# ecrireme/ESR-NeRF

Hardware: AMD Instinct MI355X
Metric: training rays/sec at 4096 rays x 128 samples (fine stage) (higher is better)
Workload: dtype f32; 1 GPU; C2: giftbox_w fine stage on the slab scene, 4096 rays x 128 samples per GPU, grid 256x256x64, s_val=20, forward + trainer loss + backward + the TV lines on every third step (no optimizer step); rays_per_gpu=4096, samples_per_ray=128, surviving_samples=524288, parallelism=dp1

## Files before the change

### esr_nerf_amd/_lib.py

```python
from __future__ import annotations

import ctypes as C
import os

import torch

_HERE = os.path.dirname(os.path.abspath(__file__))
LIB_PATH = os.path.join(_HERE, "libesr_hip.so")
LIB_PATH = os.environ.get("ESR_LIB_PATH", LIB_PATH)
ABI_VERSION = 29
_lib = None


class EsrScene(C.Structure):
    _fields_ = [
        ("xyz_min", C.c_float * 3), ("xyz_max", C.c_float * 3),
        ("mask_min", C.c_float * 3), ("mask_max", C.c_float * 3),
        ("gx", C.c_int32), ("gy", C.c_int32), ("gz", C.c_int32),
        ("mx", C.c_int32), ("my", C.c_int32), ("mz", C.c_int32),
        ("near_", C.c_float), ("stepdist", C.c_float), ("voxel_size", C.c_float),
        ("act_shift", C.c_float), ("mask_thres", C.c_float), ("fast_thres", C.c_float),
        ("s_val", C.c_float), ("max_steps", C.c_int32), ("grad_feat", C.c_float * 4),
    ]


class EsrPlan(C.Structure):
    _fields_ = [(n, C.c_int32) for n in
                ("n_on", "n_off", "tiles_on", "tiles_all", "m0", "m1", "m2", "overflow")]


class EsrFeatArgs(C.Structure):
    _fields_ = [(n, C.c_void_p) for n in ("rays_o", "rays_d", "viewdirs", "rec_ray", "rec_step", "rec_sdf",
                                          "pts", "pt_viewdirs", "pt_sdf")] + \
               [("n_pts", C.c_int32), ("sdf", C.c_void_p), ("color_on", C.c_void_p * 3),
                ("color_off", C.c_void_p * 3), ("tiles_on", C.c_int32), ("tiles_all", C.c_int32)]


class EsrFeatBwdSrc(C.Structure):
    _fields_ = [("dX", C.c_void_p), ("grad_color_on", C.c_void_p), ("grad_color_off", C.c_void_p),
                ("t0", C.c_int32), ("t1", C.c_int32)]


class EsrLtsArgs(C.Structure):
    _fields_ = [("n_pts", C.c_int32), ("n_rays", C.c_int32), ("n_sg", C.c_int32), ("pdra_mode", C.c_int32)] + \
               [(n, C.c_void_p) for n in ("base", "rough", "metal", "normal", "view", "dirs", "off_m", "emo_m",
                                          "last2", "mus", "lambdas", "lobes", "emission", "umask")]


class EsrLtsGather(C.Structure):
    _fields_ = [(n, C.c_void_p) for n in ("jp", "ray64", "pts_all", "eg", "rec_sdf", "viewdirs", "brdf_a", "emit_a",
                                          "umask_rays")] + [("n_pts", C.c_int32)] + \
               [(n, C.c_void_p) for n in ("pts2", "vd2", "sdf2", "normal", "base", "rough", "metal", "emis", "umask", "pt1")]


class EsrActJob(C.Structure):
    _fields_ = [("z", C.c_void_p), ("g_tile", C.c_void_p), ("out", C.c_void_p), ("tiles", C.c_int32), ("rows", C.c_int32),
                ("n_ch", C.c_int32), ("act", C.c_int32), ("bwd", C.c_int32), ("src", C.c_void_p), ("src_c", C.c_int32),
                ("n_src", C.c_int32), ("inv", C.c_void_p), ("pt1", C.c_void_p), ("ex", C.c_void_p * 3),
                ("ex_c", C.c_int32 * 3), ("ex_col0", C.c_int32 * 3)]


class EsrGatherJob(C.Structure):
    _fields_ = [("src", C.c_void_p), ("tile_rows", C.c_int32), ("row_stride", C.c_int32), ("col0", C.c_int32),
                ("n_ch", C.c_int32), ("perm", C.c_void_p), ("n", C.c_int32), ("out", C.c_void_p)]


class EsrPairJob(C.Structure):
    _fields_ = [("a", C.c_void_p), ("b", C.c_void_p), ("rows", C.c_int64), ("cols", C.c_int32), ("row_mask", C.c_void_p),
                ("mask_value", C.c_int32), ("count_dev", C.c_void_p), ("kind", C.c_int32), ("w_value", C.c_float),
                ("w_a", C.c_float), ("w_b", C.c_float), ("ga", C.c_void_p), ("gb", C.c_void_p)]


class EsrLtsGrads(C.Structure):
    _fields_ = [(n, C.c_void_p) for n in ("d_off_m", "d_emo_m", "d_last2", "d_base", "d_rough", "d_metal",
                                          "d_emission", "d_mus", "d_lambdas", "d_lobes")]


class EsrCdIndex(C.Structure):
    _fields_ = [("origin", C.c_double * 3), ("h", C.c_double), ("dims", C.c_int32 * 3), ("coarse", C.c_int32),
                ("cap", C.c_int64), ("keys", C.c_void_p), ("cells", C.c_void_p), ("start", C.c_void_p), ("pts", C.c_void_p),
                ("ids", C.c_void_p), ("ccap", C.c_int64), ("ckeys", C.c_void_p)]


class EsrDvgo(C.Structure):
    _fields_ = [("density", C.c_void_p), ("off_color", C.c_void_p), ("emo_color", C.c_void_p), ("dims", C.c_int32 * 3),
                ("xyz_min", C.c_float * 3), ("xyz_max", C.c_float * 3)] + \
               [(n, C.c_float) for n in ("near_", "far_", "step_scale", "interval", "act_shift")] + [("n_samples", C.c_int32)]


class EsrDvgoRays(C.Structure):
    _fields_ = [(n, C.c_void_p) for n in ("rays_o", "rays_d", "nrm", "jitter", "em_modes")] + \
               [("em_all", C.c_int32), ("n_rays", C.c_int64)]


class EsrDvgoOut(C.Structure):
    _fields_ = [(n, C.c_void_p) for n in ("alpha", "alphainv_cum", "weights", "raw_rgb", "rgb", "depth", "disp", "white_bg",
                                          "off_rgb", "on_rgb", "emo_rgb")]


class EsrDvgoBwd(C.Structure):
    _fields_ = [(n, C.c_void_p) for n in ("alpha", "alphainv_cum", "raw_rgb", "g_alphainv_cum", "g_weights", "g_raw_rgb",
                                          "g_rgb", "grad_density", "grad_off", "grad_emo")]


class EsrMlpWeights(C.Structure):
    _fields_ = [("w", C.c_void_p * 4), ("b", C.c_void_p * 4)]


class EsrWgradJob(C.Structure):
    _fields_ = [("kind", C.c_int32), ("color_row0", C.c_int32), ("t0", C.c_int32), ("t1", C.c_int32),
                ("X", C.c_void_p), ("H", C.c_void_p), ("dZ", C.c_void_p), ("dz", C.c_void_p),
                ("gw", C.c_void_p), ("gb", C.c_void_p), ("X16", C.c_void_p), ("amax", C.c_void_p)]


EXPORTS = [
    "esr_abi_version", "esr_build_info",
    "esr_sample_count", "esr_sample_fill", "esr_alpha2weight_fwd", "esr_alpha2weight_bwd",
    "esr_tv_add_grad", "esr_segment_sum",
    "esr_sample_count_f64", "esr_sample_fill_f64", "esr_alpha2weight_fwd_f64", "esr_alpha2weight_bwd_f64",
    "esr_infer_t_minmax", "esr_infer_n_samples", "esr_infer_ray_start_dir", "esr_sample_ndc_pts", "esr_sample_bg_pts",
    "esr_maskcache_lookup", "esr_raw2alpha", "esr_raw2alpha_bwd", "esr_tv_add_grad_masked",
    "esr_fine_march_count", "esr_fine_plan_begin", "esr_fine_plan", "esr_fine_plan_totals", "esr_fine_plan_offsets", "esr_fine_march_fill",
    "esr_fine_march_bwd", "esr_fine_march_bwd_rec", "esr_fine_march_cache_floats", "esr_fine_march_count_cached",
    "esr_fine_march_fill_cached", "esr_fine_march_bwd_cached", "esr_fine_march_count_ga", "esr_fine_march_fill_ga", "esr_fine_march_bwd_ga",
    "esr_fine_feat_fwd", "esr_fine_feat_fwd_x16", "esr_fine_feat_x16_bytes", "esr_fine_feat_bwd",
    "esr_mlp_packed_floats", "esr_mlp_pack", "esr_mlp_pack_batch", "esr_mlp_packed_split_elems", "esr_mlp_split_gain_offset", "esr_mlp_split_range_flag", "esr_mlp_fwd_split", "esr_mlp_fwd_fine_split", "esr_mlp_dgrad_split", "esr_mlp_dgrad_fine_split", "esr_absmax", "esr_mlp_fwd", "esr_mlp_fwd_mixed", "esr_mlp_fwd_fine", "esr_mlp_dgrad_fine", "esr_mlp_fwd_fine_bf16", "esr_mlp_dgrad_fine_bf16", "esr_mlp_dgrad", "esr_mlp_wgrad", "esr_mlp_wgrad_batch", "esr_tone_wgrad_scratch_floats", "esr_tone_wgrad_recompute", "esr_tone_wgrad_recompute_bf16", "esr_tone_wgrad_recompute_split",
    "esr_mlp_wgrad_scratch_floats",
    "esr_fine_tone_in_fwd", "esr_fine_composite_fwd", "esr_fine_composite_bwd",
    "esr_fine_tone_in_bwd", "esr_fine_loss_fwd_bwd_dp",
    "esr_expgrad_fwd", "esr_expgrad_bwd", "esr_lts_dirs", "esr_lts_ref_order", "esr_lts_perturb", "esr_lts_gather_rows",
    "esr_lts_gather_points", "esr_lts_combine_fwd", "esr_lts_combine_bwd",
    "esr_act_fwd", "esr_act_bwd", "esr_act_batch", "esr_lts_gather_rows_batch", "esr_pair_loss_batch", "esr_lts_ref_order_inv", "esr_lts_dirs_rays", "esr_composite3_fwd", "esr_composite3_bwd", "esr_lts_tone_in_bwd",
    "esr_sample_points", "esr_pair_loss_fwd_bwd", "esr_emit_edit",
    "esr_gauss3d_fwd", "esr_gauss3d_bwd", "esr_central_grad_fwd", "esr_central_grad_bwd",
    "esr_coarse_march_count", "esr_coarse_march_fill", "esr_coarse_march_bwd", "esr_coarse_march_count_ga", "esr_coarse_march_fill_ga", "esr_coarse_march_bwd_ga",
    "esr_coarse_feat_fwd", "esr_coarse_feat_bwd", "esr_coarse_shade_fwd", "esr_coarse_shade_bwd",
    "esr_adam_step", "esr_eval_aux", "esr_eval_disp",
    "esr_mlp_packed_bf16_elems", "esr_mlp_pack_bf16", "esr_mlp_fwd_bf16", "esr_mlp_dgrad_bf16", "esr_mlp_wgrad_bf16",
    "esr_brick_floats", "esr_brick_flags", "esr_brick_pack", "esr_brick_unpack", "esr_brick_list", "esr_brick_list_scratch_ints",
    "esr_smooth_grad_tv_fwd", "esr_smooth_grad_tv_bwd", "esr_host_choice_noreplace", "esr_host_choice_start", "esr_host_choice_wait",
    "esr_mesh_field", "esr_mesh_blocks", "esr_mesh_count", "esr_mesh_emit",
    "esr_cd_sample_count", "esr_cd_sample_fill", "esr_cd_cell_keys", "esr_cd_hash_insert", "esr_cd_downsample_round",
    "esr_cd_nn",
    "esr_dvgo_fwd", "esr_dvgo_eval", "esr_dvgo_bwd", "esr_dvgo_count", "esr_dvgo_count_add",
]


def lib() -> C.CDLL:
    global _lib
    if _lib is None:
        if not os.path.exists(LIB_PATH):
            raise RuntimeError(
                f"{LIB_PATH} is missing: build it with `python -m esr_nerf_amd.build` "
                "(there is no CPU fallback for the HIP path)")
        L = C.CDLL(LIB_PATH)
        L.esr_abi_version.restype = C.c_int
        L.esr_build_info.restype = C.c_char_p
        if hasattr(L, "esr_mlp_packed_floats"):
            L.esr_mlp_packed_floats.restype = C.c_int64
            L.esr_mlp_wgrad_scratch_floats.restype = C.c_int64
            L.esr_tone_wgrad_scratch_floats.restype = C.c_int64
            L.esr_fine_march_cache_floats.restype = C.c_int64
        if hasattr(L, "esr_fine_feat_x16_bytes"):
            L.esr_fine_feat_x16_bytes.restype = C.c_int64
        if hasattr(L, "esr_brick_list_scratch_ints"):
            L.esr_brick_list_scratch_ints.restype = C.c_int64
        if hasattr(L, "esr_mlp_packed_bf16_elems"):
            L.esr_mlp_packed_bf16_elems.restype = C.c_int64
        if hasattr(L, "esr_mlp_packed_split_elems"):
            L.esr_mlp_packed_split_elems.restype = C.c_int64
        if hasattr(L, "esr_mlp_split_gain_offset"):
            L.esr_mlp_split_gain_offset.restype = C.c_int64
        if hasattr(L, "esr_mesh_blocks"):
            L.esr_mesh_blocks.restype = C.c_int64
        for name in ("esr_cd_sample_count", "esr_cd_sample_fill", "esr_cd_cell_keys", "esr_cd_hash_insert",
                     "esr_cd_downsample_round", "esr_cd_nn"):
            if hasattr(L, name):
                getattr(L, name).restype = C.c_int
        if L.esr_abi_version() != ABI_VERSION:
            raise RuntimeError("libesr_hip.so ABI version mismatch: rebuild")
        _lib = L
    return _lib


def check(code: int, what: str):
    if code != 0:
        raise RuntimeError(f"{what} failed with code {code}" +
                           (" (hipError)" if code > 0 else
                            " (a capacity limit of the kernels is exceeded, include/esr_hip.h: ESR_ECAP)" if code == -2 else
                            " (bad argument)"))


def ptr(t):
    if t is None:
        return C.c_void_p(0)
    if not t.is_cuda:
        raise RuntimeError("esr_hip ops need device tensors (got a CPU tensor)")
    if not t.is_contiguous():
        raise RuntimeError("esr_hip ops need contiguous tensors")
    return C.c_void_p(t.data_ptr())


_dev_index = {}


def stream_ptr(device=None):
    idx = _dev_index.get(device)
    if idx is None:
        idx = torch.cuda.current_device() if device is None else torch.device(device).index
        if idx is None:
            idx = torch.cuda.current_device()
        elif device is not None:
            _dev_index[device] = idx
    return C.c_void_p(torch._C._cuda_getCurrentRawStream(idx))


def ptr_array(tensors, n=None):
    n = n or len(tensors)
    arr = (C.c_void_p * n)()
    for i, t in enumerate(tensors):
        arr[i] = 0 if t is None else t.data_ptr()
    return arr
```

### esr_nerf_amd/build.py

```python
from __future__ import annotations

import concurrent.futures as cf
import hashlib
import os
import shlex
import subprocess
import sys

HERE = os.path.dirname(os.path.abspath(__file__))
CSRC = os.path.join(HERE, "csrc")
OBJ = os.path.join(HERE, "_obj")
LIB = os.path.join(HERE, "libesr_hip.so")
HEADER = os.path.join(os.path.dirname(HERE), "include", "esr_hip.h")
VARIANTS = os.path.join(os.path.dirname(HERE), "tools", "_variants")
HIPCC = os.environ.get("HIPCC", "/opt/rocm/bin/hipcc")
ARCH = "gfx950"
NO_PACKED_FP32 = ["-Xclang", "-target-feature", "-Xclang", "-packed-fp32-ops"]
FLAGS = ["-O3", "-std=c++17", "-fPIC", f"--offload-arch={ARCH}", "-fvisibility=hidden",
         "-Wall", "-Wno-unused-function", "-fno-fast-math", *NO_PACKED_FP32]


EXTRA = {"tone_wgrad.hip": ["-fno-slp-vectorize"], "mlp_split.hip": ["-mllvm", "-amdgpu-mfma-vgpr-form=1"]}


def hipcc_cmd(src, extra=()):
    return [HIPCC, *FLAGS, *EXTRA.get(src, []), *extra]


def sources():
    return sorted(f for f in os.listdir(CSRC) if f.endswith(".hip"))


def _make(src, out, args):
    h = hashlib.sha1(" ".join(hipcc_cmd(src, args)[1:]).encode())
    for p in sorted([os.path.join(CSRC, src), HEADER] + [os.path.join(CSRC, f) for f in os.listdir(CSRC) if f.endswith(".h")]):
        with open(p, "rb") as f:
            h.update(f.read())
    stamp, sfile = h.hexdigest(), out + ".stamp"
    if os.path.exists(out) and os.path.exists(sfile) and open(sfile).read() == stamp:
        return False
    r = subprocess.run([*hipcc_cmd(src, args), os.path.join(CSRC, src), "-o", out], capture_output=True, text=True)
    if r.returncode != 0:
        raise RuntimeError(f"hipcc failed for {src}:\n{r.stdout}\n{r.stderr}")
    noise = ("'-packed-fp32-ops' is not a recognized feature", "argument unused during compilation: '--hip-link'")
    err = "\n".join(l for l in r.stderr.splitlines() if not any(n in l for n in noise))
    if err.strip():
        sys.stderr.write(err + "\n")
    with open(sfile, "w") as f:
        f.write(stamp)
    return True


def _compile(src, extra=(), obj=None):
    obj = obj or os.path.join(OBJ, src[:-4] + ".o")
    return obj, _make(src, obj, [*extra, "-c"])


def _link(objs, lib):
    r = subprocess.run([HIPCC, "-shared", "-fPIC", f"--offload-arch={ARCH}", "-o", lib, *objs], capture_output=True, text=True)
    if r.returncode != 0:
        raise RuntimeError(f"link failed:\n{r.stdout}\n{r.stderr}")


def build_lib(force: bool = False, jobs: int = 4) -> str:
    os.makedirs(OBJ, exist_ok=True)
    if force:
        for f in os.listdir(OBJ):
            os.remove(os.path.join(OBJ, f))
    with cf.ThreadPoolExecutor(max_workers=jobs) as ex:
        res = list(ex.map(_compile, sources()))
    if any(changed for _, changed in res) or not os.path.exists(LIB):
        _link([o for o, _ in res], LIB)
    return LIB


def build_variant(name, src, extra=()) -> str:
    if src not in sources():
        raise ValueError(f"no source csrc/{src}")
    build_lib()
    os.makedirs(VARIANTS, exist_ok=True)
    obj, _ = _compile(src, extra, os.path.join(VARIANTS, name + ".o"))
    lib = os.path.join(VARIANTS, name + ".so")
    _link([obj if s == src else os.path.join(OBJ, s[:-4] + ".o") for s in sources()], lib)
    return lib


def device_asm(src) -> str:
    os.makedirs(OBJ, exist_ok=True)
    out = os.path.join(OBJ, src[:-4] + ".s")
    _make(src, out, ["-S", "--cuda-device-only"])
    return out


if __name__ == "__main__":
    args = sys.argv[1:]
    if args[:1] == ["--variant"] and len(args) >= 3:
        print(build_variant(args[1], args[2], args[3:]))
    elif args[:1] == ["--flags"] and len(args) == 2:
        print(shlex.join(hipcc_cmd(args[1])[1:]))
    elif args in ([], ["--force"]):
        print(build_lib(force=bool(args)))
    else:
        sys.exit(__doc__)
```

### esr_nerf_amd/fine_engine.py

```python
from __future__ import annotations

import ctypes as C
import functools
import math
import os
from dataclasses import dataclass
from typing import Dict, List, Optional

import torch

from . import _lib

KIND_RADIANCE, KIND_TONEMAP = 0, 1
HID = 192
X_ROWS, DX_ROWS, XT_ROWS = 104, 64, 48


def make_scene(xyz_min, xyz_max, mask_min, mask_max, world_size, mask_size, near, stepdist,
               voxel_size, act_shift, mask_thres, fast_thres, s_val, grad_feat) -> _lib.EsrScene:
    sc = _lib.EsrScene()
    for i in range(3):
        sc.xyz_min[i], sc.xyz_max[i] = float(xyz_min[i]), float(xyz_max[i])
        sc.mask_min[i], sc.mask_max[i] = float(mask_min[i]), float(mask_max[i])
    sc.gx, sc.gy, sc.gz = [int(v) for v in world_size]
    sc.mx, sc.my, sc.mz = [int(v) for v in mask_size]
    sc.near_, sc.stepdist, sc.voxel_size = float(near), float(stepdist), float(voxel_size)
    sc.act_shift, sc.mask_thres, sc.fast_thres = float(act_shift), float(mask_thres), float(fast_thres)
    sc.s_val = float(s_val)
    diag = math.sqrt(sum((float(xyz_max[i]) - float(xyz_min[i])) ** 2 for i in range(3)))
    sc.max_steps = int(diag / float(stepdist)) + 4
    if len(grad_feat) != 4:
        raise NotImplementedError("the HIP feature kernel is built for 4 stencil radii (cfg grad_feat)")
    for i in range(4):
        sc.grad_feat[i] = float(grad_feat[i])
    return sc


_RANGE_FLAGS = {}


@dataclass
class FineCtx:
    scene: _lib.EsrScene
    n_rays: int
    tiles_on: int
    tiles_all: int
    counts: Dict[str, int]
    rays_o: torch.Tensor
    rays_d: torch.Tensor
    viewdirs: torch.Tensor
    off3: torch.Tensor
    mask_density: torch.Tensor
    sdf: torch.Tensor
    feat_args: object = None
    march_cache: object = None
    x16: bool = False
    f32_only: bool = False


class _Workspace:

    def __init__(self, device):
        self.device = device
        self.cap_tiles = 0
        self.buf: Dict[str, torch.Tensor] = {}

    ROWS = dict(X=X_ROWS, gnorm=4, H0=HID, H1=HID, H2=HID, z_off=4, z_emo=4, lin=4, Xt=XT_ROWS, Ht=HID,
                zt=4, rgb=4, dzt=4, dZt=HID, dXt=DX_ROWS, dz=4, dZ0=HID, dZ1=HID, dZ2=HID, dX=DX_ROWS,
                dweight=1, rec_w=1, rec_sdf=1, dsdf=1)

    def ensure(self, tiles: int):
        if tiles <= self.cap_tiles:
            return
        cap = int(max(tiles, self.cap_tiles) * 1.25) + 64
        self.buf = {k: torch.empty(cap * r * 32, dtype=torch.float32, device=self.device)
                    for k, r in self.ROWS.items()}
        for k in ("M0", "M1", "M2", "Mt"):
            self.buf[k] = torch.empty(cap * 3 * 64, dtype=torch.int32, device=self.device)
        self.buf["rec_ray"] = torch.empty(cap * 32, dtype=torch.int32, device=self.device)
        self.buf["rec_step"] = torch.empty(cap * 32, dtype=torch.int32, device=self.device)
        self.buf["X16"] = torch.empty(cap * 26 * 256, dtype=torch.uint8, device=self.device)
        self.cap_tiles = cap

    def __getitem__(self, k):
        return self.buf[k]


class _F32Only:
    def __init__(self, eng):
        self.eng = eng

    def __enter__(self):
        self.keep, self.eng.split_fwd = self.eng.split_fwd, False

    def __exit__(self, *exc):
        self.eng.split_fwd = self.keep
        return False


def _follows_forward(backward):
    @functools.wraps(backward)
    def run(self, ctx, *args, **kw):
        if ctx.f32_only and self.split_fwd:
            with self.f32_only():
                return backward(self, ctx, *args, **kw)
        return backward(self, ctx, *args, **kw)
    return run


class _PackGroup:
    def __init__(self, eng):
        self.eng = eng

    def __enter__(self):
        self.eng._pack_pending = []

    def __exit__(self, et, ev, tb):
        eng = self.eng
        jobs, eng._pack_pending = eng._pack_pending, None
        if et is None and jobs:
            eng._pack_flush(jobs)
        return False


class FineEngine:
    def __init__(self, device, mlp_dtype: str = "f32"):
        if mlp_dtype not in ("f32", "bf16"):
            raise ValueError("mlp_dtype must be 'f32' or 'bf16'")
        self.device = torch.device(device)
        self.bf16 = mlp_dtype == "bf16"
        self.packed16: Dict[str, torch.Tensor] = {}
        self._p16: Dict[int, C.c_void_p] = {}
        self.L = _lib.lib()
        self.ws = _Workspace(self.device)
        self.plan_dev = torch.zeros(8, dtype=torch.int32, device=self.device)
        self.plan_host = torch.zeros(8, dtype=torch.int32).pin_memory()
        self.packed = {
            k: torch.empty(self.L.esr_mlp_packed_floats(kind), dtype=torch.float32, device=self.device)
            for k, kind in (("off", KIND_RADIANCE), ("emo", KIND_RADIANCE), ("tone", KIND_TONEMAP))}
        self.ray_bufs: Dict[int, Dict[str, torch.Tensor]] = {}
        self.wgrad_scratch = torch.empty(self.L.esr_mlp_wgrad_scratch_floats(), dtype=torch.float32,
                                         device=self.device)
        self._timing = False
        self._only = None
        self._events = []
        self.n_calls = 0
        self.overlap_wgrad = True
        self._side = None
        self._raw: Dict[str, tuple] = {}
        self._pack_cache: Dict[str, tuple] = {}
        self._pack_pending = None
        self._pack_batch_cache = None
        self.x16 = self.bf16
        self.split_fwd = (not self.bf16) and os.environ.get("ESR_SPLIT_FWD", "1") != "0"
        self.split_strict = os.environ.get("ESR_SPLIT_STRICT", "0") == "1"
        self.split_fallback_steps = 0
        self.packed_split: Dict[str, torch.Tensor] = {}
        self._psplit = {}
        self.range_flag = None
        self._range_host = None
        self._range_event = None
        if self.split_fwd:
            key = str(self.device)
            if key not in _RANGE_FLAGS:
                _RANGE_FLAGS[key] = torch.zeros(1, dtype=torch.int32, device=self.device)
            self.range_flag = _RANGE_FLAGS[key]
            self._range_host = torch.zeros(1, dtype=torch.int32).pin_memory()
            with torch.cuda.device(self.device):
                _lib.check(self.L.esr_mlp_split_range_flag(_lib.ptr(self.range_flag)), "esr_mlp_split_range_flag")
        self.tone_scratch = torch.empty(self.L.esr_tone_wgrad_scratch_floats(), dtype=torch.float32, device=self.device)
        self.neus_grad = False

    def _s(self):
        return _lib.stream_ptr(self.device)

    defer_overflow = False
    overflow_seen = False
    range_strict_seen = False
    _range_streak = 0

    split_kinds = split_kinds_bwd = frozenset({0, 1, 2, 3})
    last_draws = None

    def _split_phase(self, on):
        if bool(on) != self.split_fwd:
            raise AttributeError("every split-fp16 launch follows split_fwd: set split_fwd instead")

    split_bwd = split_wgrad = split_tone_wgrad = property(lambda self: self.split_fwd, _split_phase)

    def _overflow(self):
        if not self.defer_overflow:
            raise RuntimeError("a ray exceeded scene.max_steps; the LDS bound of the march kernel is wrong")
        self.overflow_seen = True

    _RANGE_MSG = ("an input, a hidden activation or a weight of an MLP left fp16's range (|x| >= 60000, |w| >= 1023, inf / NaN) in a "
                  "split-fp16 kernel (csrc/mlp_split.hip)")

    def range_probe(self):
        if self.range_flag is None or not self.split_fwd:
            self._range_event = None
            return
        self._range_host.copy_(self.range_flag, non_blocking=True)
        self._range_event = torch.cuda.Event()
        self._range_event.record()

    def range_hit(self) -> bool:
        ev, self._range_event = self._range_event, None
        if ev is None:
            return False
        ev.synchronize()
        if int(self._range_host[0]) == 0:
            self._range_streak = 0
            return False
        self.range_flag.zero_()
        if self.split_strict:
            if self.defer_overflow:
                self.overflow_seen = True
                self.range_strict_seen = True
                return False
            raise RuntimeError(self._RANGE_MSG + " (ESR_SPLIT_STRICT=1: no fallback)")
        import warnings
        if self.split_fallback_steps == 0:
            warnings.warn(self._RANGE_MSG + ": the step is re-run on the f32 MFMA kernels (slower; counted in "
                          "engine.split_fallback_steps)", RuntimeWarning, stacklevel=3)
        self.split_fallback_steps += 1
        self._range_streak += 1
        if self._range_streak >= self.RANGE_STREAK_MAX and self.split_fwd:
            self.split_fwd = False
            warnings.warn(f"{self.RANGE_STREAK_MAX} consecutive steps left fp16's range: this engine now runs every MLP launch on the "
                          "f32 MFMA kernels (as with ESR_SPLIT_FWD=0)", RuntimeWarning, stacklevel=3)
        return True

    RANGE_STREAK_MAX = 3

    def f32_only(self):
        return _F32Only(self)

    def healed(self, run, rerun=None):
        self._range_event = None
        out = run()
        if self.range_hit():
            with self.f32_only():
                out = (rerun or run)()
        return out

    def _run(self, name, fn, *args):
        self.n_calls += 1
        if self._timing and (self._only is None or name in self._only):
            e0 = torch.cuda.Event(enable_timing=True)
            e1 = torch.cuda.Event(enable_timing=True)
            e0.record()
            rc = fn(*args)
            e1.record()
            self._events.append((name, e0, e1))
        else:
            rc = fn(*args)
        _lib.check(rc, name)

    def enable_timing(self, on: bool, only=None):
        self._timing = bool(on)
        self._only = set(only) if only is not None else None
        self._events = []

    def timing_summary(self):
        torch.cuda.synchronize(self.device)
        out = {}
        for name, e0, e1 in self._events:
            n, ms = out.get(name, (0, 0.0))
            out[name] = (n + 1, ms + e0.elapsed_time(e1))
        return out

    def _march(self, name, which, sp, rays_o, rays_d, viewdirs, *rest):
        if self.neus_grad:
            fn = getattr(self.L, f"esr_fine_march_{which}_ga")
            self._run(name, fn, sp, _lib.ptr(rays_o), _lib.ptr(rays_d), _lib.ptr(viewdirs), *rest)
        else:
            self._run(name, getattr(self.L, f"esr_fine_march_{which}"), sp, _lib.ptr(rays_o), _lib.ptr(rays_d), *rest)

    def _ray_buf(self, n, scene=None):
        if n not in self.ray_bufs:
            self.ray_bufs[n] = dict(
                cnt3=torch.empty(n, dtype=torch.int32, device=self.device),
                off3=torch.empty(n, dtype=torch.int32, device=self.device),
                stats=torch.empty(n * 3, dtype=torch.int32, device=self.device))
        rb = self.ray_bufs[n]
        if scene is not None:
            need = int(self.L.esr_fine_march_cache_floats(C.byref(scene), n))
            if rb.get("cache") is None or rb["cache"].numel() < need:
                rb["cache"] = torch.empty(need, dtype=torch.float32, device=self.device)
        return rb

    def pack(self, which: str, kind: int, weights: List[torch.Tensor], biases: List[torch.Tensor]):
        self._raw[which] = (list(weights), list(biases))
        key = tuple((t.data_ptr(), t.dtype, t.numel(), t.is_contiguous()) for t in weights) + \
            tuple((t.data_ptr(), t.dtype, t.numel(), t.is_contiguous()) for t in biases)
        hit = self._pack_cache.get(which)
        if hit is None or hit[0] != key or hit[1] != kind or hit[6] != self.packed[which].data_ptr():
            w = _lib.EsrMlpWeights()
            for i, (a, b) in enumerate(zip(weights, biases)):
                if not (a.is_cuda and b.is_cuda and a.is_contiguous() and b.is_contiguous()
                        and a.dtype == torch.float32 and b.dtype == torch.float32):
                    raise RuntimeError("MLP parameters must be contiguous fp32 device tensors")
                w.w[i], w.b[i] = a.data_ptr(), b.data_ptr()
            p32 = _lib.ptr(self.packed[which])
            p16 = None
            if self.bf16:
                n16 = self.L.esr_mlp_packed_bf16_elems(kind)
                if which not in self.packed16 or self.packed16[which].numel() != n16:
                    self.packed16[which] = torch.empty(n16, dtype=torch.bfloat16, device=self.device)
                p16 = _lib.ptr(self.packed16[which])
                self._p16[self.packed[which].data_ptr()] = p16
            if self.split_fwd and kind in self.split_kinds:
                ns = self.L.esr_mlp_packed_split_elems(kind)
                if which not in self.packed_split or self.packed_split[which].numel() != ns:
                    self.packed_split[which] = torch.empty(ns, dtype=torch.float16, device=self.device)
                self._psplit[self.packed[which].data_ptr()] = _lib.ptr(self.packed_split[which])
            hit = self._pack_cache[which] = (key, kind, w, C.byref(w), p32, p16, self.packed[which].data_ptr())
        _, _, w, wref, p32, p16, _ = hit
        if self._pack_pending is not None:
            self._pack_pending.append((which, kind, w, p32, p16))
            return
        if self.split_fwd and kind in self.split_kinds:
            return self._pack_flush([(which, kind, w, p32, p16)])
        s = self._s()
        self._run(f"mlp_pack({which})", self.L.esr_mlp_pack, kind, wref, p32, s)
        if self.bf16:
            self._run(f"mlp_pack16({which})", self.L.esr_mlp_pack_bf16, kind, wref, p16, s)

    def packing(self):
        return _PackGroup(self)

    def _pack_flush(self, jobs):
        split = [(self.packed_split[which].data_ptr() if (self.split_fwd and kind in self.split_kinds) else 0)
                 for which, kind, _, _, _ in jobs]
        sig = tuple((which, kind, C.addressof(w), p32.value, p16.value if p16 is not None else 0, sp)
                    for (which, kind, w, p32, p16), sp in zip(jobs, split))
        hit = self._pack_batch_cache
        if hit is None or hit[0] != sig:
            n = len(jobs)
            kinds = (C.c_int32 * n)(*[k for _, k, _, _, _ in jobs])
            ws = (C.c_void_p * n)(*[C.addressof(w) for _, _, w, _, _ in jobs])
            p32s = (C.c_void_p * n)(*[p.value for _, _, _, p, _ in jobs])
            p16s = (C.c_void_p * n)(*[(p.value if p is not None else 0) for _, _, _, _, p in jobs]) if self.bf16 else None
            psp = (C.c_void_p * n)(*split) if any(split) else None
            hit = self._pack_batch_cache = (sig, n, kinds, ws, p32s, p16s, psp)
        _, n, kinds, ws, p32s, p16s, psp = hit
        self._run("mlp_pack(all)", self.L.esr_mlp_pack_batch, n, kinds, ws, p32s, p16s, psp, self._s())

    def mlp_fwd(self, kind, packed, *rest):
        if not self.bf16:
            planes = self._psplit.get(packed.value) if self.split_fwd else None
            if planes is not None:
                return self.L.esr_mlp_fwd_split(kind, packed, planes, *rest)
            return self.L.esr_mlp_fwd(kind, packed, *rest)
        return self.L.esr_mlp_fwd_bf16(kind, packed, self._p16[packed.value], *rest)

    def mlp_dgrad(self, kind, packed, *rest):
        if not self.bf16:
            planes = self._psplit.get(packed.value) if self.split_fwd else None
            if planes is not None:
                return self.L.esr_mlp_dgrad_split(kind, planes, *rest[:-1], None, rest[-1])
            return self.L.esr_mlp_dgrad(kind, packed, *rest)
        return self.L.esr_mlp_dgrad_bf16(kind, self._p16[packed.value], *rest)

    def mlp_wgrad(self, *args):
        return (self.L.esr_mlp_wgrad_bf16 if self.bf16 else self.L.esr_mlp_wgrad)(*args)

    def _H(self, names):
        return _lib.ptr_array([self.ws[n] for n in names])

    def feat_args(self, rays_o, rays_d, viewdirs, sdf, tiles_on, tiles_all, color_on, color_off, ws=None):
        ws = ws or self.ws
        fa = _lib.EsrFeatArgs()
        fa.rays_o, fa.rays_d, fa.viewdirs = rays_o.data_ptr(), rays_d.data_ptr(), viewdirs.data_ptr()
        fa.rec_ray, fa.rec_step, fa.rec_sdf = ws["rec_ray"].data_ptr(), ws["rec_step"].data_ptr(), ws["rec_sdf"].data_ptr()
        fa.sdf = sdf.data_ptr()
        for g in range(3):
            fa.color_on[g] = color_on[g].data_ptr() if color_on[g] is not None else None
            fa.color_off[g] = color_off[g].data_ptr() if color_off[g] is not None else None
        fa.tiles_on, fa.tiles_all = tiles_on, tiles_all
        return fa

    def forward(self, scene, rays_o, rays_d, viewdirs, em_modes, mask_density, sdf, off_color, emo_color, prelude=None,
                heal: bool = True):
        run = lambda: self._forward(scene, rays_o, rays_d, viewdirs, em_modes, mask_density, sdf, off_color, emo_color, prelude)
        return self.healed(run) if heal else run()

    def _forward(self, scene, rays_o, rays_d, viewdirs, em_modes, mask_density, sdf, off_color, emo_color, prelude=None):
        L, s, ws = self.L, self._s(), self.ws
        n = rays_o.shape[0]
        for t in (rays_o, rays_d, viewdirs):
            if t.dtype != torch.float32:
                raise RuntimeError("rays must be fp32")
        if em_modes.dtype != torch.int64:
            raise RuntimeError("em_modes must be int64")
        cached = not self.neus_grad
        rb = self._ray_buf(n, scene if cached else None)
        last = torch.empty(n, dtype=torch.float32, device=self.device)
        n3 = (3 * n + 3) // 4 * 4
        zb = torch.zeros(8 + 2 * n3 + 4, dtype=torch.float32, device=self.device)
        plan_dev = zb[:8].view(torch.int32)
        srgb, lin = zb[8: 8 + 3 * n].view(n, 3), zb[8 + n3: 8 + n3 + 3 * n].view(n, 3)
        self._loss_acc = zb[8 + 2 * n3: 8 + 2 * n3 + 2]
        self._amax = zb[8 + 2 * n3 + 3: 8 + 2 * n3 + 4]
        self._amax_t = zb[8 + 2 * n3 + 2: 8 + 2 * n3 + 3]
        sp = C.byref(scene)
        main = torch.cuda.current_stream(self.device)
        if cached:
            self._run("march_count", L.esr_fine_march_count_cached, sp, _lib.ptr(rays_o), _lib.ptr(rays_d), _lib.ptr(mask_density),
                      _lib.ptr(sdf), n, _lib.ptr(rb["cnt3"]), _lib.ptr(last), _lib.ptr(rb["stats"]), _lib.ptr(plan_dev),
                      _lib.ptr(rb["cache"]), s)
        else:
            self._march("march_count", "count", sp, rays_o, rays_d, viewdirs, _lib.ptr(mask_density),
                        _lib.ptr(sdf), n, _lib.ptr(rb["cnt3"]), _lib.ptr(last), _lib.ptr(rb["stats"]), _lib.ptr(plan_dev), s)
        self._run("plan_totals", L.esr_fine_plan_totals, _lib.ptr(rb["cnt3"]), _lib.ptr(em_modes), _lib.ptr(rb["stats"]), n,
                  _lib.ptr(plan_dev), s)
        self.plan_host.copy_(plan_dev, non_blocking=True)
        landed = torch.cuda.Event()
        landed.record()
        self._run("plan", L.esr_fine_plan_offsets, _lib.ptr(rb["cnt3"]), _lib.ptr(em_modes), n, _lib.ptr(rb["off3"]), _lib.ptr(plan_dev), s)
        e_pre = None
        if prelude is not None:
            side = self._side_stream(0)
            side.wait_event(landed)
            with torch.cuda.stream(side):
                prelude()
                e_pre = torch.cuda.Event()
                e_pre.record(side)
        pre_rec = ws.buf.get("rec_ray")
        if pre_rec is not None:
            pre_rec.fill_(-1)
        landed.synchronize()
        n_on, n_off, _, _, m0, m1, m2, overflow = [int(v) for v in self.plan_host.tolist()]
        tiles_on = (n_on + 31) // 32
        tiles_all = tiles_on + (n_off + 31) // 32
        if overflow & 1:
            self._overflow()
        ctx = FineCtx(scene=scene, n_rays=n, tiles_on=tiles_on, tiles_all=tiles_all,
                      counts=dict(m0=m0, m1=m1, m2=m2, m3=n_on + n_off, n_on=n_on, n_off=n_off),
                      rays_o=rays_o, rays_d=rays_d, viewdirs=viewdirs, off3=rb["off3"], mask_density=mask_density, sdf=sdf,
                      f32_only=not self.bf16 and not self.split_fwd)
        if tiles_all == 0:
            if e_pre is not None:
                main.wait_event(e_pre)
            self.range_probe()
            return ctx, last, srgb, lin
        ws.ensure(tiles_all)
        if ws["rec_ray"] is not pre_rec:
            ws["rec_ray"][: tiles_all * 32].fill_(-1)
        if cached:
            self._run("march_fill", L.esr_fine_march_fill_cached, sp, _lib.ptr(rays_o), _lib.ptr(rays_d), n, _lib.ptr(rb["off3"]),
                      _lib.ptr(rb["stats"]), _lib.ptr(rb["cache"]), _lib.ptr(ws["rec_ray"]), _lib.ptr(ws["rec_step"]),
                      _lib.ptr(ws["rec_w"]), _lib.ptr(ws["rec_sdf"]), s)
            ctx.march_cache = (rb["stats"], last, rb["cache"])
        else:
            self._march("march_fill", "fill", sp, rays_o, rays_d, viewdirs, _lib.ptr(mask_density),
                        _lib.ptr(sdf), n, _lib.ptr(rb["off3"]), _lib.ptr(ws["rec_ray"]), _lib.ptr(ws["rec_step"]),
                        _lib.ptr(ws["rec_w"]), _lib.ptr(ws["rec_sdf"]), s)
        fa = self.feat_args(rays_o, rays_d, viewdirs, sdf, tiles_on, tiles_all,
                            color_on=(emo_color, off_color, None), color_off=(off_color, None, None))
        x16 = self.x16 and all(0.0 <= float(r) <= 2.0 for r in scene.grad_feat)
        ctx.x16 = x16
        ctx.amax, ctx.amax_t = self._amax, self._amax_t
        if x16:
            self._run("feat_fwd", L.esr_fine_feat_fwd_x16, sp, C.byref(fa), _lib.ptr(ws["X"]), _lib.ptr(ws["gnorm"]),
                      _lib.ptr(ws["X16"]), s)
        else:
            self._run("feat_fwd", L.esr_fine_feat_fwd, sp, C.byref(fa), _lib.ptr(ws["X"]), _lib.ptr(ws["gnorm"]), s)
        ctx.feat_args = fa
        H, M = self._H(["H0", "H1", "H2"]), self._H(["M0", "M1", "M2"])
        if e_pre is not None:
            main.wait_event(e_pre)
        if not self.bf16 and self.split_fwd and "off" in self.packed_split and "emo" in self.packed_split:
            self._run("mlp_fwd(rad)", L.esr_mlp_fwd_fine_split, _lib.ptr(self.packed["off"]), _lib.ptr(self.packed_split["off"]),
                      _lib.ptr(self.packed["emo"]), _lib.ptr(self.packed_split["emo"]), _lib.ptr(ws["X"]), tiles_on, tiles_all,
                      H, M, 88, _lib.ptr(ws["z_off"]), _lib.ptr(ws["z_emo"]), s)
        elif not self.bf16:
            self._run("mlp_fwd(rad)", L.esr_mlp_fwd_fine, _lib.ptr(self.packed["off"]), _lib.ptr(self.packed["emo"]),
                      _lib.ptr(ws["X"]), tiles_on, tiles_all, H, M, 88, _lib.ptr(ws["z_off"]), _lib.ptr(ws["z_emo"]), s)
        else:
            po, pe = _lib.ptr(self.packed["off"]), _lib.ptr(self.packed["emo"])
            self._run("mlp_fwd(rad)", L.esr_mlp_fwd_fine_bf16, po, self._p16[po.value], pe, self._p16[pe.value], _lib.ptr(ws["X"]),
                      _lib.ptr(ws["X16"]) if x16 else None, tiles_on, tiles_all, H, M, 88, _lib.ptr(ws["z_off"]),
                      _lib.ptr(ws["z_emo"]), s)
        self._run("tone_in_fwd", L.esr_fine_tone_in_fwd, _lib.ptr(ws["z_off"]), _lib.ptr(ws["z_emo"]), tiles_on, tiles_all,
                                          _lib.ptr(ws["lin"]), _lib.ptr(ws["Xt"]), s)
        self._run("mlp_fwd(tone)", self.mlp_fwd, KIND_TONEMAP, _lib.ptr(self.packed["tone"]), _lib.ptr(ws["Xt"]), 0, tiles_all,
                                 self._H(["Ht"]), self._H(["Mt"]), 2, 0, _lib.ptr(ws["zt"]), s)
        self.range_probe()
        self._run("composite_fwd", L.esr_fine_composite_fwd, _lib.ptr(ws["zt"]), _lib.ptr(ws["lin"]), _lib.ptr(ws["rec_ray"]),
                                            _lib.ptr(ws["rec_w"]), tiles_all, _lib.ptr(ws["rgb"]),
                                            _lib.ptr(srgb), _lib.ptr(lin), s)
        return ctx, last, srgb, lin

    @torch.no_grad()
    def evaluate(self, *args):
        return self.healed(lambda: self._evaluate(*args))

    def _evaluate(self, scene, rays_o, rays_d, viewdirs, mask_density, sdf, off_color, emo_color, pos_rt, far,
                  em_mode: int):
        L, s, ws, dev = self.L, self._s(), self.ws, self.device
        n = rays_o.shape[0]
        rb = self._ray_buf(n)
        last = torch.empty(n, dtype=torch.float32, device=dev)
        sp = C.byref(scene)
        em0 = torch.zeros(n, dtype=torch.int64, device=dev)
        self._run("plan_begin", L.esr_fine_plan_begin, _lib.ptr(self.plan_dev), s)
        self._march("march_count", "count", sp, rays_o, rays_d, viewdirs, _lib.ptr(mask_density),
                    _lib.ptr(sdf), n, _lib.ptr(rb["cnt3"]), _lib.ptr(last), _lib.ptr(rb["stats"]), _lib.ptr(self.plan_dev), s)
        self._run("plan", L.esr_fine_plan, _lib.ptr(rb["cnt3"]), _lib.ptr(em0), _lib.ptr(rb["stats"]), n, _lib.ptr(rb["off3"]),
                  _lib.ptr(self.plan_dev), s)
        self.plan_host.copy_(self.plan_dev, non_blocking=True)
        torch.cuda.current_stream(dev).synchronize()
        _, _, _, T, m0, m1, m2, overflow = [int(v) for v in self.plan_host.tolist()]
        if overflow & 1:
            raise RuntimeError("a ray exceeded scene.max_steps; the LDS bound of the march kernel is wrong")
        z3 = lambda: torch.zeros(n, 3, dtype=torch.float32, device=dev)
        out = {f"{sp_}/{v}_rgb": z3() for v in ("off", "on", "emo") for sp_ in ("srgb", "lin")}
        normal_m, depth3 = z3(), z3()
        depth = torch.zeros(n, dtype=torch.float32, device=dev)
        disp = torch.empty(n, dtype=torch.float32, device=dev)
        if T:
            ws.ensure(T)
            ws["rec_ray"][: T * 32].fill_(-1)
            self._march("march_fill", "fill", sp, rays_o, rays_d, viewdirs, _lib.ptr(mask_density),
                        _lib.ptr(sdf), n, _lib.ptr(rb["off3"]), _lib.ptr(ws["rec_ray"]), _lib.ptr(ws["rec_step"]),
                        _lib.ptr(ws["rec_w"]), _lib.ptr(ws["rec_sdf"]), s)
            fa = self.feat_args(rays_o, rays_d, viewdirs, sdf, 0, T, color_on=(None, None, None),
                                color_off=(off_color, emo_color, None))
            self._run("feat_fwd", L.esr_fine_feat_fwd, sp, C.byref(fa), _lib.ptr(ws["X"]), _lib.ptr(ws["gnorm"]), s)
            H, M = self._H(["H0", "H1", "H2"]), self._H(["M0", "M1", "M2"])
            for net, crow, z in (("off", 0, "z_off"), ("emo", 88, "z_emo")):
                self._run(f"mlp_fwd({net})", self.mlp_fwd, KIND_RADIANCE, _lib.ptr(self.packed[net]), _lib.ptr(ws["X"]), 0, T,
                          H, M, 0, crow, _lib.ptr(ws[z]), s)
            for name, za, zb, ton in (("off", "z_off", "z_emo", 0), ("emo", "z_emo", "z_emo", 0), ("on", "z_off", "z_emo", T)):
                self._run("tone_in_fwd", L.esr_fine_tone_in_fwd, _lib.ptr(ws[za]), _lib.ptr(ws[zb]), ton, T,
                          _lib.ptr(ws["lin"]), _lib.ptr(ws["Xt"]), s)
                self._run("mlp_fwd(tone)", self.mlp_fwd, KIND_TONEMAP, _lib.ptr(self.packed["tone"]), _lib.ptr(ws["Xt"]), 0, T,
                          self._H(["Ht"]), self._H(["Mt"]), 0, 0, _lib.ptr(ws["zt"]), s)
                self._run("composite_fwd", L.esr_fine_composite_fwd, _lib.ptr(ws["zt"]), _lib.ptr(ws["lin"]),
                          _lib.ptr(ws["rec_ray"]), _lib.ptr(ws["rec_w"]), T, _lib.ptr(ws["rgb"]),
                          _lib.ptr(out[f"srgb/{name}_rgb"]), _lib.ptr(out[f"lin/{name}_rgb"]), s)
            aux = torch.empty(T * 8 * 32, dtype=torch.float32, device=dev)
            rt = (C.c_float * 9)(*[float(v) for v in pos_rt.detach().cpu().reshape(-1).tolist()])
            self._run("eval_aux", L.esr_eval_aux, _lib.ptr(ws["X"]), X_ROWS, 40, 36, 32, _lib.ptr(ws["rec_ray"]),
                      _lib.ptr(ws["rec_step"]), T, rt, C.c_float(scene.stepdist), _lib.ptr(aux), s)
            self._run("composite3_fwd(normal)", L.esr_composite3_fwd, _lib.ptr(aux), 8, _lib.ptr(ws["rec_ray"]),
                      _lib.ptr(ws["rec_w"]), T, _lib.ptr(normal_m), s)
            self._run("composite3_fwd(depth)", L.esr_composite3_fwd, C.c_void_p(aux.data_ptr() + 4 * 32 * 4), 8,
                      _lib.ptr(ws["rec_ray"]), _lib.ptr(ws["rec_w"]), T, _lib.ptr(depth3), s)
        self._run("eval_disp", L.esr_eval_disp, _lib.ptr(depth3), _lib.ptr(last), C.c_float(far), n, _lib.ptr(depth),
                  _lib.ptr(disp), s)
        self.range_probe()
        out.update({"etc/depth": depth, "etc/disp": disp, "etc/normal": normal_m, "etc/white_bg": last.unsqueeze(-1)})
        pick = "off" if int(em_mode) == 0 else "on"
        out["srgb/rgb"], out["lin/rgb"] = out[f"srgb/{pick}_rgb"], out[f"lin/{pick}_rgb"]
        self.last_eval_counts = dict(m0=m0, m1=m1, m2=m2, tiles=T)
        return out

    @_follows_forward
    def backward(self, ctx: FineCtx, g_last, g_srgb, g_lin, grads: Dict[str, Optional[torch.Tensor]],
                 after_grids=None):
        L, ws = self.L, self.ws
        sp = C.byref(ctx.scene)
        to, ta = ctx.tiles_on, ctx.tiles_all
        g_last, g_srgb, g_lin = g_last.contiguous(), g_srgb.contiguous(), g_lin.contiguous()
        main = torch.cuda.current_stream(self.device)
        s = self._s()
        dweight = ws["dweight"] if ta > 0 else torch.zeros(32, dtype=torch.float32, device=self.device)
        overlap = self.overlap_wgrad and ta > 0
        split = not self.bf16 and self.split_fwd

        fold = ta > 0 and not self.neus_grad and grads.get("sdf") is not None

        def march_bwd(s_):
            if fold and ctx.march_cache is not None:
                st, la, ca = ctx.march_cache
                self._run("march_bwd", L.esr_fine_march_bwd_cached, sp, _lib.ptr(ctx.rays_o), _lib.ptr(ctx.rays_d), ctx.n_rays,
                          _lib.ptr(ctx.off3), _lib.ptr(st), _lib.ptr(la), _lib.ptr(ca), _lib.ptr(dweight), _lib.ptr(g_last),
                          _lib.ptr(grads["sdf"]), _lib.ptr(ws["dsdf"]), 0, s_)
                return
            if fold:
                self._run("march_bwd", L.esr_fine_march_bwd_rec, sp, _lib.ptr(ctx.rays_o), _lib.ptr(ctx.rays_d),
                          _lib.ptr(ctx.mask_density), _lib.ptr(ctx.sdf), ctx.n_rays, _lib.ptr(ctx.off3), _lib.ptr(dweight),
                          _lib.ptr(g_last), _lib.ptr(grads["sdf"]), _lib.ptr(ws["dsdf"]), 0, s_)
                return
            self._march("march_bwd", "bwd", sp, ctx.rays_o, ctx.rays_d, ctx.viewdirs, _lib.ptr(ctx.mask_density),
                        _lib.ptr(ctx.sdf), ctx.n_rays, _lib.ptr(ctx.off3), _lib.ptr(dweight), _lib.ptr(g_last),
                        _lib.ptr(grads["sdf"]), s_)

        def feat_bwd(s_):
            src = (_lib.EsrFeatBwdSrc * 1)()
            src[0].dX = ws["dX"].data_ptr()
            src[0].grad_color_on = grads["emo_color"].data_ptr()
            src[0].grad_color_off = grads["off_color"].data_ptr()
            src[0].t0, src[0].t1 = 0, ta
            self._run("feat_bwd", L.esr_fine_feat_bwd, sp, C.byref(ctx.feat_args), _lib.ptr(ws["X"]),
                      _lib.ptr(ws["gnorm"]), src, 1, _lib.ptr(ws["dsdf"]) if fold else None, _lib.ptr(grads["sdf"]),
                      None, None, 0, s_)

        def tone_wgrad(s_):
            (w0, w1), (b0, _) = self._raw["tone"]
            if split:
                self._run("tone_wgrad", L.esr_tone_wgrad_recompute_split, _lib.ptr(ws["Xt"]), _lib.ptr(ws["dzt"]), _lib.ptr(w0.detach()),
                          _lib.ptr(b0.detach()), _lib.ptr(w1.detach()), _lib.ptr(ctx.amax_t), 0, ta, _lib.ptr(grads["tone_w"][0]),
                          _lib.ptr(grads["tone_b"][0]), _lib.ptr(grads["tone_w"][1]), _lib.ptr(grads["tone_b"][1]),
                          _lib.ptr(self.tone_scratch), C.c_int64(self.tone_scratch.numel()), s_)
                return
            self._run("tone_wgrad", L.esr_tone_wgrad_recompute_bf16 if self.bf16 else L.esr_tone_wgrad_recompute,
                      _lib.ptr(ws["Xt"]), _lib.ptr(ws["dzt"]), _lib.ptr(w0.detach()),
                      _lib.ptr(b0.detach()), _lib.ptr(w1.detach()), 0, ta, _lib.ptr(grads["tone_w"][0]),
                      _lib.ptr(grads["tone_b"][0]), _lib.ptr(grads["tone_w"][1]), _lib.ptr(grads["tone_b"][1]),
                      _lib.ptr(self.tone_scratch), C.c_int64(self.tone_scratch.numel()), s_)

        def wgrads(s_):
            tone_wgrad(s_)
            Hh, dZh = self._H(["H0", "H1", "H2"]), self._H(["dZ0", "dZ1", "dZ2"])
            keep = [Hh, dZh]
            todo = [(KIND_RADIANCE, ws["X"], Hh, dZh, ws["dz"], 0, to, "emo_w", "emo_b"),
                    (KIND_RADIANCE, ws["X"], Hh, dZh, ws["dz"], to, ta, "off_w", "off_b")]
            jobs = (_lib.EsrWgradJob * len(todo))()
            for j, (kind, X, Hs, dZs, dzs, r0, r1, gwk, gbk) in enumerate(todo):
                gwa, gba = _lib.ptr_array(grads[gwk]), _lib.ptr_array(grads[gbk])
                keep += [gwa, gba]
                jb = jobs[j]
                jb.kind, jb.color_row0, jb.t0, jb.t1 = kind, 0, r0, r1
                jb.X, jb.dz = X.data_ptr(), dzs.data_ptr()
                jb.H, jb.dZ = C.addressof(Hs), C.addressof(dZs)
                jb.gw, jb.gb = C.addressof(gwa), C.addressof(gba)
                if ctx.x16:
                    jb.X16 = ws["X16"].data_ptr()
                if split:
                    jb.amax = ctx.amax.data_ptr()
            self._run("mlp_wgrad(all)", L.esr_mlp_wgrad_batch, jobs, len(todo), 1 if self.bf16 else 0,
                      _lib.ptr(self.wgrad_scratch), C.c_int64(self.wgrad_scratch.numel()), s_)

        if ta == 0:
            march_bwd(s)
            if after_grids is not None:
                after_grids()
            return
        self._run("composite_bwd", L.esr_fine_composite_bwd, _lib.ptr(g_srgb), _lib.ptr(g_lin), _lib.ptr(ws["rgb"]),
                  _lib.ptr(ws["lin"]), _lib.ptr(ws["rec_ray"]), _lib.ptr(ws["rec_w"]), ta, _lib.ptr(ws["dweight"]),
                  _lib.ptr(ws["dzt"]), s)
        if fold:
            march_bwd(s)
        dZt_arg = _lib.ptr_array([None])
        M = self._H(["M0", "M1", "M2"])
        dZ = self._H(["dZ0", "dZ1", "dZ2"])
        if self.bf16:
            self._run("mlp_dgrad(tone)", L.esr_mlp_dgrad_bf16, KIND_TONEMAP, self._p16[self.packed["tone"].data_ptr()],
                      _lib.ptr(ws["dzt"]), 0, ta, self._H(["Mt"]), dZt_arg, _lib.ptr(ws["dXt"]), s)
        elif split:
            self._run("mlp_dgrad(tone)", L.esr_mlp_dgrad_split, KIND_TONEMAP, _lib.ptr(self.packed_split["tone"]), _lib.ptr(ws["dzt"]),
                      0, ta, self._H(["Mt"]), dZt_arg, _lib.ptr(ws["dXt"]), _lib.ptr(ctx.amax_t), s)
        else:
            self._run("mlp_dgrad(tone)", L.esr_mlp_dgrad, KIND_TONEMAP, _lib.ptr(self.packed["tone"]), _lib.ptr(ws["dzt"]), 0, ta,
                      self._H(["Mt"]), dZt_arg, _lib.ptr(ws["dXt"]), s)
        self._run("tone_in_bwd", L.esr_fine_tone_in_bwd, _lib.ptr(ws["dXt"]), _lib.ptr(ws["Xt"]), _lib.ptr(g_lin), _lib.ptr(ws["lin"]),
                  _lib.ptr(ws["z_off"]), _lib.ptr(ws["z_emo"]), _lib.ptr(ws["rec_ray"]), _lib.ptr(ws["rec_w"]), to, ta,
                  _lib.ptr(ws["dz"]), s)
        if self.bf16:
            pe, po = self.packed["emo"].data_ptr(), self.packed["off"].data_ptr()
            self._run("mlp_dgrad(rad)", L.esr_mlp_dgrad_fine_bf16, self._p16[pe], self._p16[po],
                      _lib.ptr(ws["dz"]), to, ta, M, dZ, _lib.ptr(ws["dX"]), s)
        elif split:
            self._run("mlp_dgrad(rad)", L.esr_mlp_dgrad_fine_split, _lib.ptr(self.packed_split["emo"]),
                      _lib.ptr(self.packed_split["off"]), _lib.ptr(ws["dz"]), to, ta, M, dZ, _lib.ptr(ws["dX"]),
                      _lib.ptr(ctx.amax), s)
        else:
            self._run("mlp_dgrad(rad)", L.esr_mlp_dgrad_fine, _lib.ptr(self.packed["emo"]), _lib.ptr(self.packed["off"]),
                      _lib.ptr(ws["dz"]), to, ta, M, dZ, _lib.ptr(ws["dX"]), s)
        if not overlap:
            feat_bwd(s)
            if not fold:
                march_bwd(s)
            if after_grids is not None:
                after_grids()
            wgrads(s)
            return
        e_dgrad = torch.cuda.Event()
        e_dgrad.record(main)
        side = self._side_stream(0)
        side.wait_event(e_dgrad)
        with torch.cuda.stream(side):
            wgrads(_lib.stream_ptr(self.device))
            e_w = torch.cuda.Event()
            e_w.record(side)
        feat_bwd(s)
        if not fold:
            march_bwd(s)
        if after_grids is not None:
            after_grids()
        main.wait_event(e_w)

    def _side_stream(self, i=0):
        if self._side is None:
            self._side = {}
        if i not in self._side:
            self._side[i] = torch.cuda.Stream(self.device)
        return self._side[i]

    def loss_fwd_bwd(self, last, srgb, lin, rgbs, white_bg=True, weight_linear=0.1, weight_entropy_last=0.001,
                     scale=1.0):
        n = last.shape[0]
        acc = getattr(self, "_loss_acc", None)
        self._loss_acc = None
        pair = acc if acc is not None and acc.device == srgb.device else torch.zeros(2, dtype=torch.float32, device=self.device)
        self.loss_pair = pair
        loss = pair[:1]
        g_srgb = torch.empty_like(srgb)
        g_lin = torch.empty_like(lin)
        g_last = torch.empty_like(last)
        self._run("loss", self.L.esr_fine_loss_fwd_bwd_dp,
                  _lib.ptr(srgb), _lib.ptr(lin), _lib.ptr(last), _lib.ptr(rgbs.contiguous()), n,
                  C.c_float(1.0 if white_bg else 0.0), C.c_float(weight_linear), C.c_float(weight_entropy_last),
                  C.c_float(scale), _lib.ptr(loss), _lib.ptr(g_srgb), _lib.ptr(g_lin), _lib.ptr(g_last), self._s())
        return loss, g_last, g_srgb, g_lin
```

### include/esr_hip.h

```cpp
#ifndef ESR_HIP_H
#define ESR_HIP_H

#include <stdint.h>

#ifdef __cplusplus
extern "C" {
#endif

#define ESR_EINVAL (-1)
#define ESR_ECAP   (-2)

#define ESR_TILE 32

#define ESR_ABI_VERSION 29
int esr_abi_version(void);
const char *esr_build_info(void);


int esr_sample_count(const float *rays_o, const float *rays_d, const float *xyz_min,
                     const float *xyz_max, float near_, float far_, float stepdist,
                     int64_t n_rays, float *t_min, float *t_max, int64_t *n_steps,
                     int64_t *cumsum, int64_t *total, void *stream);

int esr_sample_fill(const float *rays_o, const float *rays_d, const float *xyz_min,
                    const float *xyz_max, const float *t_min, const int64_t *cumsum,
                    float stepdist, int64_t n_rays, int64_t total, float *ray_pts,
                    uint8_t *mask_outbbox, int64_t *ray_id, int64_t *step_id, void *stream);

int esr_alpha2weight_fwd(const float *alpha, const int64_t *ray_id, int64_t n_pts,
                         int64_t n_rays, float *weight, float *T, float *alphainv_last,
                         int64_t *i_start, int64_t *i_end, void *stream);

int esr_alpha2weight_bwd(const float *alpha, const float *weight, const float *T,
                         const float *alphainv_last, const int64_t *i_start,
                         const int64_t *i_end, int64_t n_pts, int64_t n_rays,
                         const float *grad_weights, const float *grad_last, float *grad,
                         void *stream);

int esr_tv_add_grad(const float *param, float *grad, float wx, float wy, float wz,
                    int64_t sz_i, int64_t sz_j, int64_t sz_k, int64_t n, int dense_mode,
                    void *stream);

int esr_segment_sum(const float *src, const int64_t *index, int64_t n, int64_t c,
                    float *out, int64_t n_seg, void *stream);

int esr_sample_count_f64(const double *rays_o, const double *rays_d, const double *xyz_min, const double *xyz_max,
                         float near_, float far_, float stepdist, int64_t n_rays, double *t_min, double *t_max,
                         int64_t *n_steps, int64_t *cumsum, int64_t *total, void *stream);
int esr_sample_fill_f64(const double *rays_o, const double *rays_d, const double *xyz_min, const double *xyz_max,
                        const double *t_min, const int64_t *cumsum, float stepdist, int64_t n_rays, int64_t total,
                        double *ray_pts, uint8_t *mask_outbbox, int64_t *ray_id, int64_t *step_id, void *stream);
int esr_alpha2weight_fwd_f64(const double *alpha, const int64_t *ray_id, int64_t n_pts, int64_t n_rays, double *weight,
                             double *T, double *alphainv_last, int64_t *i_start, int64_t *i_end, void *stream);
int esr_alpha2weight_bwd_f64(const double *alpha, const double *weight, const double *T, const double *alphainv_last,
                             const int64_t *i_start, const int64_t *i_end, int64_t n_pts, int64_t n_rays,
                             const double *grad_weights, const double *grad_last, double *grad, void *stream);

int esr_infer_t_minmax(const float *rays_o, const float *rays_d, const float *xyz_min, const float *xyz_max,
                       float near_, float far_, int64_t n_rays, float *t_min, float *t_max, void *stream);
int esr_infer_n_samples(const float *rays_d, const float *t_min, const float *t_max, float stepdist, int64_t n_rays,
                        int64_t *n_samples, void *stream);
int esr_infer_ray_start_dir(const float *rays_o, const float *rays_d, const float *t_min, int64_t n_rays,
                            float *rays_start, float *rays_dir, void *stream);
int esr_sample_ndc_pts(const float *rays_o, const float *rays_d, const float *xyz_min, const float *xyz_max,
                       int32_t n_samples, int64_t n_rays, float *rays_pts, uint8_t *mask_outbbox, void *stream);
int esr_sample_bg_pts(const float *rays_o, const float *rays_d, const float *t_max, float bg_preserve, int32_t n_samples,
                      int64_t n_rays, float *rays_pts, void *stream);
int esr_maskcache_lookup(const uint8_t *world, const float *xyz, const float *xyz2ijk_scale, const float *xyz2ijk_shift,
                         int32_t sz_i, int32_t sz_j, int32_t sz_k, int64_t n_pts, uint8_t *out, void *stream);
int esr_raw2alpha(const float *density, float shift, float interval, const float *interval_per_point, int64_t n_pts,
                  float *exp_d, float *alpha, void *stream);
int esr_raw2alpha_bwd(const float *exp_d, const float *grad_back, float interval, const float *interval_per_point,
                      int64_t n_pts, float *grad, void *stream);
int esr_tv_add_grad_masked(const float *param, float *grad, const float *mask, float wx, float wy, float wz,
                           int64_t sz_i, int64_t sz_j, int64_t sz_k, int64_t n, int dense_mode, void *stream);


typedef struct esr_scene {
    float xyz_min[3], xyz_max[3];
    float mask_min[3], mask_max[3];
    int32_t gx, gy, gz;
    int32_t mx, my, mz;
    float near_, stepdist, voxel_size;
    float act_shift, mask_thres;
    float fast_thres;
    float s_val;
    int32_t max_steps;
    float grad_feat[4];
} esr_scene_t;

typedef struct esr_plan {
    int32_t n_on;
    int32_t n_off;
    int32_t tiles_on;
    int32_t tiles_all;
    int32_t m0, m1, m2;
    int32_t overflow;
} esr_plan_t;

int esr_fine_march_count(const esr_scene_t *scene, const float *rays_o, const float *rays_d,
                         const float *mask_density, const float *sdf, int32_t n_rays,
                         int32_t *cnt3, float *alphainv_last, int32_t *ray_stats, esr_plan_t *plan,
                         void *stream);

int esr_fine_plan_begin(esr_plan_t *plan, void *stream);

int esr_fine_plan(const int32_t *cnt3, const int64_t *em_modes, const int32_t *ray_stats,
                  int32_t n_rays, int32_t *off3, esr_plan_t *plan, void *stream);
int esr_fine_plan_totals(const int32_t *cnt3, const int64_t *em_modes, const int32_t *ray_stats, int32_t n_rays,
                         esr_plan_t *plan, void *stream);
int esr_fine_plan_offsets(const int32_t *cnt3, const int64_t *em_modes, int32_t n_rays, int32_t *off3, esr_plan_t *plan,
                          void *stream);

int esr_fine_march_fill(const esr_scene_t *scene, const float *rays_o, const float *rays_d,
                        const float *mask_density, const float *sdf, int32_t n_rays,
                        const int32_t *off3, int32_t *rec_ray, int32_t *rec_step,
                        float *rec_w, float *rec_sdf, void *stream);

int esr_fine_march_bwd(const esr_scene_t *scene, const float *rays_o, const float *rays_d,
                       const float *mask_density, const float *sdf, int32_t n_rays,
                       const int32_t *off3, const float *dweight, const float *dlast,
                       float *grad_sdf, void *stream);

int esr_fine_march_bwd_rec(const esr_scene_t *scene, const float *rays_o, const float *rays_d,
                           const float *mask_density, const float *sdf, int32_t n_rays,
                           const int32_t *off3, const float *dweight, const float *dlast,
                           float *grad_sdf, float *dsdf_rec, int32_t accumulate, void *stream);

int64_t esr_fine_march_cache_floats(const esr_scene_t *scene, int32_t n_rays);
int esr_fine_march_count_cached(const esr_scene_t *scene, const float *rays_o, const float *rays_d,
                                const float *mask_density, const float *sdf, int32_t n_rays, int32_t *cnt3,
                                float *alphainv_last, int32_t *ray_stats, esr_plan_t *plan, float *cache, void *stream);
int esr_fine_march_fill_cached(const esr_scene_t *scene, const float *rays_o, const float *rays_d, int32_t n_rays,
                               const int32_t *off3, const int32_t *ray_stats, const float *cache,
                               int32_t *rec_ray, int32_t *rec_step, float *rec_w, float *rec_sdf, void *stream);
int esr_fine_march_bwd_cached(const esr_scene_t *scene, const float *rays_o, const float *rays_d, int32_t n_rays,
                              const int32_t *off3, const int32_t *ray_stats, const float *alphainv_last,
                              const float *cache, const float *dweight, const float *dlast, float *grad_sdf,
                              float *dsdf_rec, int32_t accumulate, void *stream);

int esr_fine_march_count_ga(const esr_scene_t *scene, const float *rays_o, const float *rays_d, const float *viewdirs,
                            const float *mask_density, const float *sdf, int32_t n_rays, int32_t *cnt3,
                            float *alphainv_last, int32_t *ray_stats, esr_plan_t *plan, void *stream);
int esr_fine_march_fill_ga(const esr_scene_t *scene, const float *rays_o, const float *rays_d, const float *viewdirs,
                           const float *mask_density, const float *sdf, int32_t n_rays, const int32_t *off3,
                           int32_t *rec_ray, int32_t *rec_step, float *rec_w, float *rec_sdf, void *stream);
int esr_fine_march_bwd_ga(const esr_scene_t *scene, const float *rays_o, const float *rays_d, const float *viewdirs,
                          const float *mask_density, const float *sdf, int32_t n_rays, const int32_t *off3,
                          const float *dweight, const float *dlast, float *grad_sdf, void *stream);

typedef struct esr_feat_args {
    const float *rays_o, *rays_d, *viewdirs;
    const int32_t *rec_ray, *rec_step;
    const float *rec_sdf;
    const float *pts, *pt_viewdirs, *pt_sdf;
    int32_t n_pts;
    const float *sdf;
    const float *color_on[3], *color_off[3];
    int32_t tiles_on, tiles_all;
} esr_feat_args_t;

int esr_fine_feat_fwd(const esr_scene_t *scene, const esr_feat_args_t *args, float *X, float *gnorm,
                      void *stream);
int64_t esr_fine_feat_x16_bytes(int32_t n_tiles);
int esr_fine_feat_fwd_x16(const esr_scene_t *scene, const esr_feat_args_t *args, float *X, float *gnorm, void *X16,
                          void *stream);

typedef struct esr_feat_bwd_src {
    const float *dX;
    float *grad_color_on, *grad_color_off;
    int32_t t0, t1;
} esr_feat_bwd_src_t;

int esr_fine_feat_bwd(const esr_scene_t *scene, const esr_feat_args_t *args, const float *X,
                      const float *gnorm, const esr_feat_bwd_src_t *src, int32_t n_src,
                      const float *dsdf_extra, float *grad_sdf, float *dsdf_out, const float *grad4,
                      int32_t grad4_mode, void *stream);

#define ESR_MLP_RADIANCE 0
#define ESR_MLP_TONEMAP  1
#define ESR_MLP_BRDF     2
#define ESR_MLP_EMIT     3
#define ESR_MLP_COARSE   4
#define ESR_MLP_MAX_LAYERS 4

typedef struct esr_mlp_weights {
    const float *w[ESR_MLP_MAX_LAYERS];
    const float *b[ESR_MLP_MAX_LAYERS];
} esr_mlp_weights_t;

int64_t esr_mlp_packed_floats(int kind);
int esr_mlp_pack(int kind, const esr_mlp_weights_t *w, float *packed, void *stream);
int esr_mlp_pack_batch(int n, const int32_t *kinds, const esr_mlp_weights_t *const *w, float *const *packed32,
                       void *const *packed16, void *const *packed_split, void *stream);
int64_t esr_mlp_packed_split_elems(int kind);
int64_t esr_mlp_split_gain_offset(int kind);
int esr_mlp_split_range_flag(uint32_t *flag);
int esr_mlp_fwd_split(int kind, const float *packed32, const void *planes, const float *X, int32_t t0, int32_t t1,
                      float *const *H, uint32_t *const *M, int save, int color_row0, float *zout, void *stream);
int esr_mlp_fwd_fine_split(const float *packed32_off, const void *planes_off, const float *packed32_emo,
                           const void *planes_emo, const float *X, int32_t t_on, int32_t t_all, float *const *H,
                           uint32_t *const *M, int color_row_detached, float *z_off, float *z_emo, void *stream);
int esr_mlp_dgrad_split(int kind, const void *planes, const float *dz, int32_t t0, int32_t t1, const uint32_t *const *M,
                        float *const *dZ, float *dX, float *amax, void *stream);
int esr_mlp_dgrad_fine_split(const void *planes_emo, const void *planes_off, const float *dz, int32_t t_on, int32_t t_all,
                             const uint32_t *const *M, float *const *dZ, float *dX, float *amax, void *stream);
int esr_absmax(const float *x, int64_t n, float *out, void *stream);

int esr_mlp_fwd(int kind, const float *packed, const float *X, int32_t t0, int32_t t1,
                float *const *H, uint32_t *const *M, int save, int color_row0, float *zout,
                void *stream);
int esr_mlp_fwd_mixed(int kind, const float *packed, const float *X, int32_t t0, int32_t t_mid, int32_t t1,
                      float *const *H, uint32_t *const *M, int color_row_detached, float *zout, void *stream);

int esr_mlp_fwd_fine(const float *packed_off, const float *packed_emo, const float *X, int32_t t_on, int32_t t_all,
                     float *const *H, uint32_t *const *M, int color_row_detached, float *z_off, float *z_emo,
                     void *stream);
int esr_mlp_dgrad_fine(const float *packed_emo, const float *packed_off, const float *dz, int32_t t_on, int32_t t_all,
                       const uint32_t *const *M, float *const *dZ, float *dX, void *stream);
int esr_mlp_fwd_fine_bf16(const float *packed32_off, const void *packed16_off, const float *packed32_emo,
                          const void *packed16_emo, const float *X, const void *X16, int32_t t_on, int32_t t_all,
                          float *const *H, uint32_t *const *M, int color_row_detached, float *z_off, float *z_emo,
                          void *stream);
int esr_mlp_dgrad_fine_bf16(const void *packed16_emo, const void *packed16_off, const float *dz, int32_t t_on, int32_t t_all,
                            const uint32_t *const *M, float *const *dZ, float *dX, void *stream);

int esr_mlp_dgrad(int kind, const float *packed, const float *dz, int32_t t0, int32_t t1,
                  const uint32_t *const *M, float *const *dZ, float *dX, void *stream);

int64_t esr_mlp_wgrad_scratch_floats(void);
int esr_mlp_wgrad(int kind, const float *X, int color_row0, const float *const *H,
                  const float *const *dZ, const float *dz, int32_t t0, int32_t t1,
                  float *const *gw, float *const *gb, float *scratch, int64_t scratch_floats,
                  void *stream);

typedef struct esr_wgrad_job {
    int32_t kind, color_row0, t0, t1;
    const float *X;
    const float *const *H;
    const float *const *dZ;
    const float *dz;
    float *const *gw;
    float *const *gb;
    const void *X16;
    const float *amax;
} esr_wgrad_job_t;
int esr_mlp_wgrad_batch(const esr_wgrad_job_t *jobs, int32_t n_jobs, int bf16_operands, float *scratch,
                        int64_t scratch_floats, void *stream);

int64_t esr_tone_wgrad_scratch_floats(void);
int esr_tone_wgrad_recompute(const float *Xt, const float *dzt, const float *W0, const float *b0, const float *W1,
                             int32_t t0, int32_t t1, float *gw0, float *gb0, float *gw1, float *gb1,
                             float *scratch, int64_t scratch_floats, void *stream);
int esr_tone_wgrad_recompute_bf16(const float *Xt, const float *dzt, const float *W0, const float *b0, const float *W1,
                                  int32_t t0, int32_t t1, float *gw0, float *gb0, float *gw1, float *gb1,
                                  float *scratch, int64_t scratch_floats, void *stream);
int esr_tone_wgrad_recompute_split(const float *Xt, const float *dzt, const float *W0, const float *b0, const float *W1,
                                   const float *amax, int32_t t0, int32_t t1, float *gw0, float *gb0, float *gw1,
                                   float *gb1, float *scratch, int64_t scratch_floats, void *stream);

int64_t esr_mlp_packed_bf16_elems(int kind);
int esr_mlp_pack_bf16(int kind, const esr_mlp_weights_t *w, void *packed16, void *stream);
int esr_mlp_fwd_bf16(int kind, const float *packed32, const void *packed16, const float *X, int32_t t0,
                     int32_t t1, float *const *H, uint32_t *const *M, int save, int color_row0,
                     float *zout, void *stream);
int esr_mlp_dgrad_bf16(int kind, const void *packed16, const float *dz, int32_t t0, int32_t t1,
                       const uint32_t *const *M, float *const *dZ, float *dX, void *stream);
int esr_mlp_wgrad_bf16(int kind, const float *X, int color_row0, const float *const *H,
                       const float *const *dZ, const float *dz, int32_t t0, int32_t t1,
                       float *const *gw, float *const *gb, float *scratch, int64_t scratch_floats,
                       void *stream);

int esr_fine_tone_in_fwd(const float *z_off, const float *z_emo, int32_t tiles_on,
                         int32_t tiles_all, float *lin, float *Xt, void *stream);

int esr_fine_composite_fwd(const float *zt, const float *lin, const int32_t *rec_ray,
                           const float *rec_w, int32_t tiles_all, float *rgb,
                           float *srgb_marched, float *lin_marched, void *stream);

int esr_fine_composite_bwd(const float *g_srgb, const float *g_lin, const float *rgb,
                           const float *lin, const int32_t *rec_ray, const float *rec_w,
                           int32_t tiles_all, float *dweight, float *dzt, void *stream);

int esr_fine_tone_in_bwd(const float *dXt, const float *Xt, const float *g_lin, const float *lin,
                         const float *z_off, const float *z_emo, const int32_t *rec_ray,
                         const float *rec_w, int32_t tiles_on, int32_t tiles_all, float *dz,
                         void *stream);

int esr_fine_loss_fwd_bwd_dp(const float *srgb_marched, const float *lin_marched,
                             const float *alphainv_last, const float *rgbs, int32_t n_rays,
                             float white_bg, float weight_linear, float weight_entropy_last, float scale,
                             float *loss, float *g_srgb, float *g_lin, float *g_last,
                             void *stream);

int esr_pair_loss_fwd_bwd(const float *a, const float *b, int64_t rows, int32_t cols,
                          const uint8_t *row_mask, int mask_value, const int32_t *count_dev,
                          int kind, float w_value, float w_a, float w_b, float *loss, float *ga,
                          float *gb, void *stream);


int esr_expgrad_fwd(const esr_scene_t *scene, const float *rays_o, const float *rays_d,
                    const int32_t *rec_ray, const int32_t *rec_step, const float *pts,
                    const float *noise, float eps, const float *sdf, int32_t n, int zero_pad,
                    float *out, void *stream);
int esr_expgrad_bwd(const esr_scene_t *scene, const float *rays_o, const float *rays_d,
                    const int32_t *rec_ray, const int32_t *rec_step, const float *pts,
                    const float *noise, float eps, const float *g, int32_t n, int zero_pad,
                    float *grad_sdf, void *stream);

int esr_lts_ref_order(const int32_t *rec_ray, const int32_t *cnt3, const int32_t *off3, const int64_t *cnt3_cumsum,
                      int32_t n_slots, int64_t *perm, int64_t *ray64, void *stream);
int esr_lts_perturb(const float *pts_all, const int64_t *perm, const float *noise_normal, const float *noise_emit,
                    float emit_eps, int32_t m3, float *noise_n, float *pts_e, void *stream);
int esr_lts_gather_rows(const float *src, int32_t tile_rows, int32_t row_stride, int32_t col0, int32_t n_ch,
                        const int64_t *perm, int32_t n, float *out, void *stream);
typedef struct esr_lts_gather {
    const int64_t *jp, *ray64;
    const float *pts_all, *eg, *rec_sdf, *viewdirs, *brdf_a, *emit_a;
    const uint8_t *umask_rays;
    int32_t n_pts;
    float *pts2, *vd2, *sdf2, *normal, *base, *rough, *metal, *emis;
    uint8_t *umask;
    int32_t *pt1;
} esr_lts_gather_t;
int esr_lts_gather_points(const esr_lts_gather_t *g, void *stream);

int esr_lts_dirs(const float *raw, const float *normal, int32_t n_pts, int32_t rays_plus_one,
                 float *dirs, void *stream);

typedef struct esr_lts_args {
    int32_t n_pts, n_rays, n_sg, pdra_mode;
    const float *base, *rough, *metal;
    const float *normal, *view;
    const float *dirs;
    const float *off_m, *emo_m, *last2;
    const float *mus, *lambdas, *lobes;
    const float *emission;
    const uint8_t *umask;
} esr_lts_args_t;

typedef struct esr_lts_grads {
    float *d_off_m, *d_emo_m, *d_last2;
    float *d_base, *d_rough, *d_metal, *d_emission;
    float *d_mus, *d_lambdas, *d_lobes;
} esr_lts_grads_t;

int esr_lts_combine_fwd(const esr_lts_args_t *args, float *off_hat, float *emo_hat, void *stream);
int esr_lts_combine_bwd(const esr_lts_args_t *args, const float *g_off_hat, const float *g_emo_hat,
                        const esr_lts_grads_t *grads, void *stream);

int esr_emit_edit(float *emit, const int64_t *em_modes, const float *em_intensities,
                  const float *em_colors, int32_t n, void *stream);

#define ESR_ACT_MAX_JOBS 4
typedef struct esr_act_job {
    const float *z;
    const float *g_tile;
    float *out;
    int32_t tiles, rows, n_ch, act, bwd;
    const float *src;
    int32_t src_c, n_src;
    const int32_t *inv;
    const int32_t *pt1;
    const float *ex[3];
    int32_t ex_c[3], ex_col0[3];
} esr_act_job_t;
int esr_act_batch(const esr_act_job_t *jobs, int32_t n_jobs, void *stream);

#define ESR_GATHER_MAX_JOBS 4
typedef struct esr_gather_job {
    const float *src;
    int32_t tile_rows, row_stride, col0, n_ch;
    const int64_t *perm;
    int32_t n;
    float *out;
} esr_gather_job_t;
int esr_lts_gather_rows_batch(const esr_gather_job_t *jobs, int32_t n_jobs, void *stream);

#define ESR_PAIR_MAX_JOBS 6
typedef struct esr_pair_job {
    const float *a, *b;
    int64_t rows;
    int32_t cols;
    const uint8_t *row_mask;
    int32_t mask_value;
    const int32_t *count_dev;
    int32_t kind;
    float w_value, w_a, w_b;
    float *ga, *gb;
} esr_pair_job_t;
int esr_pair_loss_batch(const esr_pair_job_t *jobs, int32_t n_jobs, float *loss, void *stream);

int esr_lts_ref_order_inv(const int32_t *rec_ray, const int32_t *cnt3, const int32_t *off3, const int64_t *cnt3_cumsum,
                          int32_t n_slots, int64_t *perm, int64_t *ray64, int32_t *inv, void *stream);

int esr_lts_dirs_rays(const float *raw, const float *normal, const float *pts, int32_t n_pts, int32_t rays_plus_one,
                      float *dirs, float *o2, float *d2, float *v_rand, void *stream);

int esr_act_fwd(const float *z, int32_t tiles, int32_t rows, int32_t n_ch, int act, float *out, void *stream);
int esr_act_bwd(const float *z, const float *g, int32_t tiles, int32_t rows, int32_t n_ch, int act,
                float *dz, void *stream);
int esr_composite3_fwd(const float *v, int32_t rows, const int32_t *rec_ray, const float *rec_w,
                       int32_t tiles, float *out, void *stream);
int esr_composite3_bwd(const float *g, const float *v, int32_t rows, const int32_t *rec_ray,
                       const float *rec_w, int32_t tiles, int accumulate, float *dv, float *dweight,
                       void *stream);
int esr_lts_tone_in_bwd(const float *dXt, const float *Xt, const float *g_lin, const float *lin, const float *z_off,
                        const float *z_emo, const int32_t *rec_ray, const float *rec_w, int32_t tiles_on,
                        int32_t tiles_all, float *dz_off, float *dz_emo, void *stream);
int esr_sample_points(const esr_scene_t *scene, const float *rays_o, const float *rays_d,
                      const int32_t *rec_ray, const int32_t *rec_step, int32_t n, float *pts, void *stream);


int esr_gauss3d_fwd(const float *in, const float *weights_host, int ksize, int32_t gx, int32_t gy,
                    int32_t gz, float *out, void *stream);
int esr_gauss3d_bwd(const float *gout, const float *weights_host, int ksize, int32_t gx, int32_t gy,
                    int32_t gz, float *gin, void *stream);

int esr_central_grad_fwd(const float *sdf, int32_t gx, int32_t gy, int32_t gz, float voxel_size,
                         float *grad, void *stream);
int esr_central_grad_bwd(const float *ggrad, int32_t gx, int32_t gy, int32_t gz, float voxel_size,
                         float *gsdf, void *stream);

int esr_coarse_march_count(const esr_scene_t *scene, const float *rays_o, const float *rays_d,
                           const float *mask_density, const float *sdf_smooth, int32_t n_rays,
                           int32_t *cnt3, float *alphainv_last, float *cum_weights, int32_t *ray_stats,
                           esr_plan_t *plan, void *stream);
int esr_coarse_march_fill(const esr_scene_t *scene, const float *rays_o, const float *rays_d,
                          const float *mask_density, const float *sdf_smooth, int32_t n_rays,
                          const int32_t *off3, int32_t *rec_ray, int32_t *rec_step, float *rec_w,
                          float *rec_sdf, void *stream);
int esr_coarse_march_bwd(const esr_scene_t *scene, const float *rays_o, const float *rays_d,
                         const float *mask_density, const float *sdf_smooth, int32_t n_rays,
                         const int32_t *off3, const float *dweight, const float *dlast,
                         float *grad_sdf_smooth, void *stream);

int esr_coarse_march_count_ga(const esr_scene_t *scene, const float *rays_o, const float *rays_d, const float *viewdirs,
                              const float *mask_density, const float *sdf_smooth, const float *gg, int32_t n_rays,
                              int32_t *cnt3, float *alphainv_last, float *cum_weights, int32_t *ray_stats,
                              esr_plan_t *plan, void *stream);
int esr_coarse_march_fill_ga(const esr_scene_t *scene, const float *rays_o, const float *rays_d, const float *viewdirs,
                             const float *mask_density, const float *sdf_smooth, const float *gg, int32_t n_rays,
                             const int32_t *off3, int32_t *rec_ray, int32_t *rec_step, float *rec_w, float *rec_sdf,
                             void *stream);
int esr_coarse_march_bwd_ga(const esr_scene_t *scene, const float *rays_o, const float *rays_d, const float *viewdirs,
                            const float *mask_density, const float *sdf_smooth, const float *gg, int32_t n_rays,
                            const int32_t *off3, const float *dweight, const float *dlast, float *grad_sdf_smooth,
                            float *grad_gg, void *stream);

int esr_coarse_feat_fwd(const esr_scene_t *scene, const float *rays_o, const float *rays_d,
                        const float *viewdirs, const int32_t *rec_ray, const int32_t *rec_step,
                        int32_t tiles_on, int32_t tiles_all, const float *grad_grid,
                        const float *off_color, const float *emo_color, float *X, float *gnorm,
                        void *stream);
int esr_coarse_feat_bwd(const esr_scene_t *scene, const float *rays_o, const float *rays_d,
                        const float *viewdirs, const int32_t *rec_ray, const int32_t *rec_step,
                        int32_t tiles_on, int32_t tiles_all, const float *X, const float *gnorm,
                        const float *dX_off, const float *dX_emo, float *g_grad_grid,
                        float *g_off_color, float *g_emo_color, void *stream);

int esr_coarse_shade_fwd(const float *z_off, const float *z_emo, const int32_t *rec_ray,
                         const float *rec_w, int32_t tiles_on, int32_t tiles_all, float *rgb,
                         float *srgb_marched, void *stream);
int esr_coarse_shade_bwd(const float *g_srgb, const float *g_white_bg, const float *rgb,
                         const float *z_off, const float *z_emo, const int32_t *rec_ray,
                         const float *rec_w, int32_t tiles_on, int32_t tiles_all, float *dz_off,
                         float *dz_emo, float *dweight, void *stream);


int esr_eval_aux(const float *X, int32_t xrows, int32_t row_nx, int32_t row_ny, int32_t row_nz,
                 const int32_t *rec_ray, const int32_t *rec_step, int32_t tiles,
                 const float *pos_rt_host, float stepdist, float *aux, void *stream);
int esr_eval_disp(const float *depth3, const float *alphainv_last, float far_, int32_t n_rays,
                  float *depth, float *disp, void *stream);


int esr_adam_step(float *param, const float *grad, float *exp_avg, float *exp_avg_sq,
                  const float *per_lr, int64_t n, float lr, float beta1, float beta2, float eps,
                  float weight_decay, int32_t step, void *stream);

int esr_smooth_grad_tv_fwd(const float *sdf, const uint8_t *mask, const float *conv_w27, float conv_bias,
                           int32_t gx, int32_t gy, int32_t gz, float voxel_size, int64_t masked_cells,
                           float weight, float *work6, float *loss, void *stream);
int esr_smooth_grad_tv_bwd(const float *work6, int32_t gx, int32_t gy, int32_t gz, float voxel_size,
                           int64_t masked_cells, float weight, const float *grad_out ,
                           float *grad_sdf, void *stream);

int esr_host_choice_noreplace(uint32_t *key, int32_t *pos, int64_t n, int64_t k, int64_t *out);
int esr_host_choice_start(uint32_t *key, int32_t *pos, int64_t n, int64_t k, int64_t *out, void **job);
int esr_host_choice_wait(void *job);


int esr_brick_floats(void);
int esr_brick_flags(const float *buf, int64_t n, uint8_t *flags, void *stream);
int esr_brick_pack(const float *buf, int64_t n, const int64_t *brick_idx, int64_t n_idx, float *packed,
                   void *stream);
int esr_brick_unpack(const float *packed, const int64_t *brick_idx, int64_t n_idx, float *buf, int64_t n,
                     void *stream);
int64_t esr_brick_list_scratch_ints(void);
int esr_brick_list(const uint8_t *flags, int64_t n_bricks, int64_t cap, int64_t *idx, int64_t *count, int32_t *scratch,
                   void *stream);


int esr_mesh_field(const float *sdf, int32_t gx, int32_t gy, int32_t gz, const float *box_host, const float *xs,
                   const float *ys, const float *zs, int32_t r0, int32_t r1, int32_t r2, float *u, void *stream);
int64_t esr_mesh_blocks(int32_t r0, int32_t r1, int32_t r2);
int esr_mesh_count(const float *u, int32_t r0, int32_t r1, int32_t r2, float threshold, int64_t *counts, void *stream);
int esr_mesh_emit(const float *u, int32_t r0, int32_t r1, int32_t r2, float threshold, const int64_t *offsets,
                  int32_t *vid, double *vertices, int64_t *triangles, void *stream);


typedef struct {
    double origin[3];
    double h;
    int32_t dims[3];
    int32_t coarse;
    int64_t cap;
    const int64_t *keys;
    const int32_t *cells;
    const int64_t *start;
    const double *pts;
    const int32_t *ids;
    int64_t ccap;
    const int64_t *ckeys;
} esr_cd_index_t;

int esr_cd_sample_count(const double *vertices, const int64_t *triangles, int64_t n_tri, double thresh, int64_t *counts,
                        void *stream);
int esr_cd_sample_fill(const double *vertices, const int64_t *triangles, int64_t n_tri, double thresh,
                       const int64_t *offsets, double *points, void *stream);
int esr_cd_cell_keys(const esr_cd_index_t *index, const double *points, int64_t n, int64_t *keys, void *stream);
int esr_cd_hash_insert(const int64_t *ukeys, int64_t n_u, int64_t cap, int64_t *table_keys, int32_t *table_vals,
                       void *stream);
int esr_cd_downsample_round(const esr_cd_index_t *index, const double *points, int64_t n, double thresh, int8_t *state,
                            int32_t *changed, void *stream);
int esr_cd_nn(const esr_cd_index_t *index, const double *queries, int64_t nq, double max_dist, double *dist, void *stream);


typedef struct {
    const float *density;
    const float *off_color;
    const float *emo_color;
    int32_t dims[3];
    float xyz_min[3];
    float xyz_max[3];
    float near_, far_, step_scale, interval, act_shift;
    int32_t n_samples;
} esr_dvgo_t;

typedef struct {
    const float *rays_o;
    const float *rays_d;
    const float *nrm;
    const float *jitter;
    const int32_t *em_modes;
    int32_t em_all;
    int64_t n_rays;
} esr_dvgo_rays_t;

typedef struct {
    float *alpha;
    float *alphainv_cum;
    float *weights;
    float *raw_rgb;
    float *rgb;
    float *depth;
    float *disp;
    float *white_bg;
    float *off_rgb;
    float *on_rgb;
    float *emo_rgb;
} esr_dvgo_out_t;

typedef struct {
    const float *alpha;
    const float *alphainv_cum;
    const float *raw_rgb;
    const float *g_alphainv_cum;
    const float *g_weights;
    const float *g_raw_rgb;
    const float *g_rgb;
    float *grad_density;
    float *grad_off;
    float *grad_emo;
} esr_dvgo_bwd_t;

int esr_dvgo_fwd(const esr_dvgo_t *model, const esr_dvgo_rays_t *rays, const esr_dvgo_out_t *out, void *stream);
int esr_dvgo_eval(const esr_dvgo_t *model, const esr_dvgo_rays_t *rays, const esr_dvgo_out_t *out, void *stream);
int esr_dvgo_bwd(const esr_dvgo_t *model, const esr_dvgo_rays_t *rays, const esr_dvgo_bwd_t *bwd, void *stream);
int esr_dvgo_count(const esr_dvgo_t *model, const esr_dvgo_rays_t *rays, float *sum, void *stream);
int esr_dvgo_count_add(const float *sum, int64_t n, float *count, void *stream);

#ifdef __cplusplus
}
#endif
#endif
```

Before: 2.071 million rays/s.

## Fuse tone-mapper input encoding and its backward into split MFMA kernels

Adds fused tone-mapper kernels that build the positional-encoded input in the forward and fold the tone_in backward (sin/cos chain rule, softplus grad, lin gradient) into the dgrad epilogue. Only the backward fused kernel is wired in by default, replacing mlp_dgrad_split plus a separate tone_in_bwd launch and skipping the dXt round trip through memory. The forward fused kernel is exported but unused. This adds register pressure and complexity in the dgrad body, and the tone net is a small part of the step.

Result: no change. 2.088 million rays/s (median of 6 runs) (+0.9%).

```diff
diff --git a/esr_nerf_amd/_lib.py b/esr_nerf_amd/_lib.py
--- a/esr_nerf_amd/_lib.py
+++ b/esr_nerf_amd/_lib.py
@@ -8,7 +8,7 @@
 _HERE = os.path.dirname(os.path.abspath(__file__))
 LIB_PATH = os.path.join(_HERE, "libesr_hip.so")
 LIB_PATH = os.environ.get("ESR_LIB_PATH", LIB_PATH)
-ABI_VERSION = 29
+ABI_VERSION = 30
 _lib = None
 
 
@@ -124,7 +124,7 @@
     "esr_fine_march_bwd", "esr_fine_march_bwd_rec", "esr_fine_march_cache_floats", "esr_fine_march_count_cached",
     "esr_fine_march_fill_cached", "esr_fine_march_bwd_cached", "esr_fine_march_count_ga", "esr_fine_march_fill_ga", "esr_fine_march_bwd_ga",
     "esr_fine_feat_fwd", "esr_fine_feat_fwd_x16", "esr_fine_feat_x16_bytes", "esr_fine_feat_bwd",
-    "esr_mlp_packed_floats", "esr_mlp_pack", "esr_mlp_pack_batch", "esr_mlp_packed_split_elems", "esr_mlp_split_gain_offset", "esr_mlp_split_range_flag", "esr_mlp_fwd_split", "esr_mlp_fwd_fine_split", "esr_mlp_dgrad_split", "esr_mlp_dgrad_fine_split", "esr_absmax", "esr_mlp_fwd", "esr_mlp_fwd_mixed", "esr_mlp_fwd_fine", "esr_mlp_dgrad_fine", "esr_mlp_fwd_fine_bf16", "esr_mlp_dgrad_fine_bf16", "esr_mlp_dgrad", "esr_mlp_wgrad", "esr_mlp_wgrad_batch", "esr_tone_wgrad_scratch_floats", "esr_tone_wgrad_recompute", "esr_tone_wgrad_recompute_bf16", "esr_tone_wgrad_recompute_split",
+    "esr_mlp_packed_floats", "esr_mlp_pack", "esr_mlp_pack_batch", "esr_mlp_packed_split_elems", "esr_mlp_split_gain_offset", "esr_mlp_split_range_flag", "esr_mlp_fwd_split", "esr_mlp_fwd_fine_split", "esr_mlp_dgrad_split", "esr_mlp_dgrad_fine_split", "esr_tone_fused_fwd", "esr_tone_fused_bwd", "esr_absmax", "esr_mlp_fwd", "esr_mlp_fwd_mixed", "esr_mlp_fwd_fine", "esr_mlp_dgrad_fine", "esr_mlp_fwd_fine_bf16", "esr_mlp_dgrad_fine_bf16", "esr_mlp_dgrad", "esr_mlp_wgrad", "esr_mlp_wgrad_batch", "esr_tone_wgrad_scratch_floats", "esr_tone_wgrad_recompute", "esr_tone_wgrad_recompute_bf16", "esr_tone_wgrad_recompute_split",
     "esr_mlp_wgrad_scratch_floats",
     "esr_fine_tone_in_fwd", "esr_fine_composite_fwd", "esr_fine_composite_bwd",
     "esr_fine_tone_in_bwd", "esr_fine_loss_fwd_bwd_dp",
diff --git a/esr_nerf_amd/build.py b/esr_nerf_amd/build.py
--- a/esr_nerf_amd/build.py
+++ b/esr_nerf_amd/build.py
@@ -20,7 +20,8 @@
          "-Wall", "-Wno-unused-function", "-fno-fast-math", *NO_PACKED_FP32]
 
 
-EXTRA = {"tone_wgrad.hip": ["-fno-slp-vectorize"], "mlp_split.hip": ["-mllvm", "-amdgpu-mfma-vgpr-form=1"]}
+EXTRA = {"tone_wgrad.hip": ["-fno-slp-vectorize"], "mlp_split.hip": ["-mllvm", "-amdgpu-mfma-vgpr-form=1"],
+         "tone_fused.hip": ["-mllvm", "-amdgpu-mfma-vgpr-form=1"]}
 
 
 def hipcc_cmd(src, extra=()):
diff --git a/esr_nerf_amd/csrc/tone_fused.hip b/esr_nerf_amd/csrc/tone_fused.hip
--- /dev/null
+++ b/esr_nerf_amd/csrc/tone_fused.hip
@@ -0,0 +1,222 @@
+#include "tone_fused_body.h"
+
+unsigned *esr_split_range_flag_ptr();
+
+namespace {
+
+constexpr int TONE = ESR_MLP_TONEMAP;
+constexpr int XT_ROWS = 48;
+
+__device__ __forceinline__ float softplus_grad(float z) { return z > 20.f ? 1.f : esr_sigmoid(z); }
+
+constexpr int ang_c(int h, int k) { return h == 0 ? (k < 5 ? 0 : k < 7 ? 2 : k == 7 ? 1 : 0) : (k < 5 ? 1 : 2); }
+constexpr int ang_i(int h, int k) { return h == 0 ? (k < 5 ? k : k < 7 ? k - 2 : 0) : (k < 5 ? k : k - 5); }
+constexpr int ang_slot(int h, int c, int i)
+{
+    for (int k = 0; k < 9; ++k)
+        if (ang_c(h, k) == c && ang_i(h, k) == i) return k;
+    return -1;
+}
+struct RowSrc { int kind, a; };
+constexpr RowSrc row_src(int h, int R)
+{
+    return R < 3 ? RowSrc{1, R}
+         : R < 18 ? RowSrc{2, ang_slot(h, (R - 3) / 5, (R - 3) % 5)}
+         : R < 33 ? RowSrc{3, ang_slot(h, (R - 18) / 5, (R - 18) % 5)} : RowSrc{0, 0};
+}
+static_assert([] {
+    for (int h = 0; h < 2; ++h)
+        for (int j = 0; j < 3; ++j)
+            for (int i = 0; i < 8; ++i)
+                if (row_src(h, 16 * j + 8 * h + i).kind >= 2 && row_src(h, 16 * j + 8 * h + i).a < 0) return false;
+    return true;
+}(), "every sin / cos row of a lane half has its angle slot");
+
+struct ToneFwdIO {
+    const float *z_off, *z_emo;
+    int tiles_on;
+    float *lin, *Xt;
+
+    template <int KIND, int N>
+    __device__ __forceinline__ void fetch_x(const SplitBatch &, const SplitSeg &, int t, bool live, int h, int s_, float (&xn)[N]) const
+    {
+        static_assert(KIND == TONE && N == 24, "the tone mapper's 48-row input tile");
+        const size_t z4 = (size_t)t * 4 * 32 + s_;
+        float v[3];
+#pragma unroll
+        for (int c = 0; c < 3; ++c) {
+            v[c] = esr_softplus(z_off[z4 + c * 32]);
+            if (t < tiles_on) v[c] = esr_softplus(z_emo[z4 + c * 32]) + v[c];
+        }
+        float sn[9], cs[9];
+#pragma unroll
+        for (int k = 0; k < 9; ++k) {
+            const float lc = h ? v[ang_c(1, k)] : v[ang_c(0, k)];
+            const float f = h ? (float)(1 << ang_i(1, k)) : (float)(1 << ang_i(0, k));
+            esr_sincos(lc * f, sn[k], cs[k]);
+        }
+        auto val = [&](RowSrc r) -> float {
+            return r.kind == 1 ? v[r.a] : r.kind == 2 ? sn[r.a] : r.kind == 3 ? cs[r.a] : 0.f;
+        };
+#pragma unroll
+        for (int j = 0; j < 3; ++j)
+#pragma unroll
+            for (int i = 0; i < 8; ++i)
+                xn[j * 8 + i] = h ? val(row_src(1, 16 * j + 8 + i)) : val(row_src(0, 16 * j + i));
+        const rsrc_t RX = make_rsrc(Xt + (size_t)t * XT_ROWS * 32, live ? XT_ROWS * 32 * 4 : 0);
+        const int xvoff = (h * 8 * 32 + s_) * 4;
+#pragma unroll
+        for (int j = 0; j < 3; ++j)
+#pragma unroll
+            for (int i = 0; i < 8; ++i) bstore1(RX, xn[j * 8 + i], xvoff, (16 * j + i) * 128);
+        const rsrc_t RL = make_rsrc(lin + (size_t)t * 4 * 32, (live && h == 0) ? 4 * 32 * 4 : 0);
+#pragma unroll
+        for (int c = 0; c < 4; ++c) bstore1(RL, c < 3 ? v[c < 3 ? c : 0] : 0.f, s_ * 4, c * 128);
+    }
+};
+
+__global__ void __launch_bounds__(64 * SPW, split_occ(TONE)) tone_fused_fwd_kernel(SplitBatch AB, ToneFwdIO io)
+{
+    split_fwd_body<TONE>(AB, io);
+}
+
+constexpr int dx_row(int it, int r, int h) { return 32 * it + acc_row(r, h); }
+constexpr int row_chan(int R) { return R < 3 ? R : R < 18 ? (R - 3) / 5 : R < 33 ? (R - 18) / 5 : -1; }
+constexpr int NFAC = 17;
+constexpr int fac_slot(int it, int r) { return it == 0 ? r : (r == 0 ? 16 : -1); }
+
+struct ToneBwdIO {
+    static constexpr bool STORE_DX = false;
+    const float *Xt, *g_lin, *z_off, *z_emo, *rec_w;
+    const int32_t *rec_ray;
+    int tiles_on;
+    float *dz;
+
+    struct State {
+        float fac[NFAC];
+        float sa[3], sb[3];
+        int ray;
+        float w, z[3];
+    };
+
+    template <int KIND>
+    __device__ __forceinline__ void group_begin(State &S, int t, int h, int s_) const
+    {
+        const rsrc_t RX = make_rsrc(Xt + (size_t)t * XT_ROWS * 32, XT_ROWS * 32 * 4);
+#pragma unroll
+        for (int it = 0; it < 2; ++it)
+#pragma unroll
+            for (int r = 0; r < 16; ++r) {
+                const int k = fac_slot(it, r);
+                if (k < 0) continue;
+                const int RA = dx_row(it, r, 0), RB = dx_row(it, r, 1);
+                auto partner = [](int R) { return R >= 3 && R < 18 ? R + 15 : R >= 18 && R < 33 ? R - 15 : 0; };
+                auto coef = [](int R) { return R >= 3 && R < 18 ? (float)(1 << ((R - 3) % 5)) : R >= 18 && R < 33 ? -(float)(1 << ((R - 18) % 5)) : 0.f; };
+                const int P = h ? partner(RB) : partner(RA);
+                const float x = bload1(RX, s_ * 4 + P * 128, 0);
+                const float fa = RA < 3 ? 1.f : coef(RA) * x, fb = RB < 3 ? 1.f : coef(RB) * x;
+                S.fac[k] = h ? fb : fa;
+            }
+#pragma unroll
+        for (int c = 0; c < 3; ++c) S.sa[c] = S.sb[c] = 0.f;
+        const int j = t * 32 + s_;
+        const size_t z4 = (size_t)t * 4 * 32 + s_;
+        S.ray = rec_ray[j];
+        S.w = rec_w[j];
+#pragma unroll
+        for (int c = 0; c < 3; ++c) S.z[c] = (t < tiles_on) ? z_emo[z4 + c * 32] : z_off[z4 + c * 32];
+    }
+
+    template <int KIND, int it, int r0>
+    __device__ __forceinline__ void dx_pair(State &S, int, float v0, float v1) const
+    {
+        add<it, r0>(S, v0);
+        add<it, r0 + 1>(S, v1);
+    }
+    template <int it, int r>
+    __device__ __forceinline__ void add(State &S, float v) const
+    {
+        constexpr int k = fac_slot(it, r), ca = row_chan(dx_row(it, r, 0)), cb = row_chan(dx_row(it, r, 1));
+        if constexpr (k >= 0 && (ca >= 0 || cb >= 0)) {
+            const float p = v * S.fac[k];
+            if constexpr (ca >= 0) S.sa[ca] += p;
+            if constexpr (cb >= 0) S.sb[cb] += p;
+        }
+    }
+
+    template <int KIND>
+    __device__ __forceinline__ void group_end(State &S, int t, bool live, int h, int s_) const
+    {
+        float d[3];
+#pragma unroll
+        for (int c = 0; c < 3; ++c) {
+            d[c] = h ? S.sb[c] : S.sa[c];
+            d[c] += __shfl_xor(d[c], 32);
+        }
+        const rsrc_t RD = make_rsrc(dz + (size_t)t * 4 * 32, (live && h == 0) ? 4 * 32 * 4 : 0);
+        const int ray = S.ray;
+#pragma unroll
+        for (int c = 0; c < 3; ++c) {
+            float o = 0.f;
+            if (ray >= 0) o = (S.w * g_lin[3 * ray + c] + d[c]) * softplus_grad(S.z[c]);
+            bstore1(RD, o, s_ * 4, c * 128);
+        }
+        bstore1(RD, 0.f, s_ * 4, 3 * 128);
+    }
+};
+
+__global__ void __launch_bounds__(64 * SPW, split_occ(TONE)) tone_fused_bwd_kernel(DSplitBatch AB, ToneBwdIO io)
+{
+    split_dgrad_body<TONE>(AB, io);
+}
+
+int tone_grid(int tiles)
+{
+    const int groups = (tiles + SPW - 1) / SPW, cap = 256 * split_occ(TONE);
+    return groups < cap ? groups : cap;
+}
+
+}
+
+ESR_API int esr_tone_fused_fwd(const float *packed32, const void *planes, const float *z_off, const float *z_emo, int32_t tiles_on,
+                               int32_t tiles_all, uint32_t *Mt, float *lin, float *Xt, float *zt, void *stream)
+{
+    if (tiles_on < 0 || tiles_all < tiles_on) return ESR_EINVAL;
+    if (tiles_all == 0) return 0;
+    if (!packed32 || !planes || !z_off || (tiles_on > 0 && !z_emo) || !Mt || !lin || !Xt || !zt) return ESR_EINVAL;
+    using S = SplitSteps<TONE>;
+    SplitBatch B = {};
+    B.M[0] = Mt;
+    B.range = esr_split_range_flag_ptr();
+    B.nseg = 1;
+    const int grid = tone_grid(tiles_all);
+    B.seg[0] = SplitSeg{packed32, static_cast<const _Float16 *>(planes), 0, tiles_all, 2, 0, zt, 0, grid};
+    static std::atomic<uint64_t> optin{0};
+    if (int rc = esr_lds_optin(reinterpret_cast<const void *>(&tone_fused_fwd_kernel), S::LDS_BYTES, optin)) return rc;
+    tone_fused_fwd_kernel<<<grid, 64 * SPW, S::LDS_BYTES, esr_stream(stream)>>>(B, ToneFwdIO{z_off, z_emo, tiles_on, lin, Xt});
+    ESR_CHECK_LAUNCH();
+    return 0;
+}
+
+ESR_API int esr_tone_fused_bwd(const void *planes, const float *dzt, const uint32_t *Mt, const float *Xt, const float *g_lin,
+                               const float *z_off, const float *z_emo, const int32_t *rec_ray, const float *rec_w, int32_t tiles_on,
+                               int32_t tiles_all, float *dz, float *amax, void *stream)
+{
+    if (tiles_on < 0 || tiles_all < tiles_on) return ESR_EINVAL;
+    if (tiles_all == 0) return 0;
+    if (!planes || !dzt || !Mt || !Xt || !g_lin || !z_off || (tiles_on > 0 && !z_emo) || !rec_ray || !rec_w || !dz) return ESR_EINVAL;
+    using S = SplitSteps<TONE, true>;
+    DSplitBatch B = {};
+    B.dz = dzt;
+    B.M[0] = Mt;
+    B.amax = amax;
+    B.nseg = 1;
+    const int grid = tone_grid(tiles_all);
+    B.seg[0] = DSplitSeg{static_cast<const _Float16 *>(planes), 0, tiles_all, 0, grid};
+    static std::atomic<uint64_t> optin{0};
+    if (int rc = esr_lds_optin(reinterpret_cast<const void *>(&tone_fused_bwd_kernel), S::WBYTES, optin)) return rc;
+    tone_fused_bwd_kernel<<<grid, 64 * SPW, S::WBYTES, esr_stream(stream)>>>(
+        B, ToneBwdIO{Xt, g_lin, z_off, z_emo, rec_w, rec_ray, tiles_on, dz});
+    ESR_CHECK_LAUNCH();
+    return 0;
+}
diff --git a/esr_nerf_amd/csrc/tone_fused_body.h b/esr_nerf_amd/csrc/tone_fused_body.h
--- /dev/null
+++ b/esr_nerf_amd/csrc/tone_fused_body.h
@@ -0,0 +1,622 @@
+#pragma once
+#include "mlp_common.h"
+
+#include <type_traits>
+
+typedef _Float16 f16x8 __attribute__((ext_vector_type(8)));
+
+#ifndef ESR_SPLIT_STAMP
+#define ESR_SPLIT_STAMP(i)
+#endif
+
+namespace {
+
+constexpr int SPW = 4;
+constexpr float SPLIT_RANGE = 60000.f;
+constexpr int WRING = 3;
+
+__device__ __forceinline__ f32x16 mfma_h(f16x8 a, f16x8 b, f32x16 c)
+{
+    return __builtin_amdgcn_mfma_f32_32x32x16_f16(a, b, c, 0, 0, 0);
+}
+
+template <int I, int N, typename F>
+__device__ __forceinline__ void sfor(F &&f)
+{
+    if constexpr (I < N) {
+        f(std::integral_constant<int, I>{});
+        sfor<I + 1, N>(f);
+    }
+}
+
+__device__ __forceinline__ void split8(const float (&v)[8], f16x8 &p1, f16x8 &p2)
+{
+#pragma unroll
+    for (int i = 0; i < 8; ++i) {
+        const _Float16 h = (_Float16)v[i];
+        p1[i] = h;
+        p2[i] = (_Float16)(v[i] - (float)h);
+    }
+}
+
+typedef _Float16 f16x2 __attribute__((ext_vector_type(2)));
+template <int I0>
+__device__ __forceinline__ void put_pair(f16x8 &dst, float a, float b)
+{
+    const f16x2 hh = {(_Float16)a, (_Float16)b};
+    unsigned u = __builtin_bit_cast(unsigned, hh);
+    asm volatile("" : "+v"(u));
+    const f16x2 pinned = __builtin_bit_cast(f16x2, u);
+    dst[I0] = pinned[0];
+    dst[I0 + 1] = pinned[1];
+}
+
+template <int I0>
+__device__ __forceinline__ void put_residual_pair(f16x8 &dst, const f16x8 &first, float v0, float v1)
+{
+    const unsigned u = __builtin_bit_cast(u32x4, first)[I0 >> 1];
+    unsigned r;
+    float d0, d1;
+    asm volatile("v_fma_mix_f32 %1, %3, -1.0, %4 op_sel_hi:[1,0,0]\n\t"
+                 "v_fma_mix_f32 %2, %3, -1.0, %5 op_sel:[1,0,0] op_sel_hi:[1,0,0]\n\t"
+                 "v_cvt_pk_f16_f32 %0, %1, %2"
+                 : "=v"(r), "=&v"(d0), "=&v"(d1) : "v"(u), "v"(v0), "v"(v1));
+    const f16x2 pinned = __builtin_bit_cast(f16x2, r);
+    dst[I0] = pinned[0];
+    dst[I0 + 1] = pinned[1];
+}
+
+template <int KIND, bool BWD = false> struct SplitSteps {
+    static constexpr SplitLayout L = BWD ? split_layout_t(KIND) : split_layout(KIND);
+    static constexpr int BASE_CHUNK = BWD ? split_layout(KIND).total_chunks : 0;
+    static constexpr int NL = L.n_layers;
+    static constexpr int n_steps()
+    {
+        int n = 0;
+        for (int l = 0; l < NL; ++l) n += L.pairs[l];
+        return n;
+    }
+    static constexpr int NS = n_steps();
+    static constexpr int layer_of(int s)
+    {
+        int l = 0;
+        while (s >= L.pairs[l]) { s -= L.pairs[l]; ++l; }
+        return l;
+    }
+    static constexpr int pair_of(int s)
+    {
+        int l = 0;
+        while (s >= L.pairs[l]) { s -= L.pairs[l]; ++l; }
+        return s;
+    }
+    static constexpr int tiles_in(int s)
+    {
+        const int l = layer_of(s), p = pair_of(s);
+        return L.tiles_out[l] - 2 * p >= 2 ? 2 : 1;
+    }
+    static constexpr int chunks(int s) { return tiles_in(s) * 2 * L.ks[layer_of(s)]; }
+    static constexpr int chunk0(int s) { return BASE_CHUNK + L.off_chunk[layer_of(s)] + pair_of(s) * 2 * 2 * L.ks[layer_of(s)]; }
+    static constexpr int max_chunks()
+    {
+        int m = 0;
+        for (int s = 0; s < NS; ++s) m = chunks(s) > m ? chunks(s) : m;
+        return m;
+    }
+    static constexpr int BUF = max_chunks() * 1024;
+    static constexpr int BIAS_FLOATS = 32 * MAX_HID_TILES;
+    static constexpr bool RES = L.total_chunks <= 64;
+    static constexpr int WBYTES = RES ? L.total_chunks * 1024 : 2 * BUF;
+    static constexpr int LDS_BYTES = WBYTES + NL * BIAS_FLOATS * 4;
+    static constexpr int PRE = (max_chunks() * 64 + 64 * SPW - 1) / (64 * SPW);
+};
+
+struct SplitSeg {
+    const float *packed32;
+    const _Float16 *planes;
+    int t0, t1, save, crow;
+    float *zout;
+    int b0, nb;
+};
+constexpr int MAX_SPLIT_SEG = 3;
+struct SplitBatch {
+    const float *X;
+    float *H[3];
+    unsigned *M[3];
+    unsigned *range;
+    int nseg;
+    SplitSeg seg[MAX_SPLIT_SEG];
+};
+
+__device__ __forceinline__ void step_barrier()
+{
+    __builtin_amdgcn_sched_barrier(0);
+    asm volatile("" ::: "memory");
+    __builtin_amdgcn_s_waitcnt(0xc07f);
+    __builtin_amdgcn_s_barrier();
+    asm volatile("" ::: "memory");
+    __builtin_amdgcn_sched_barrier(0);
+}
+
+constexpr int split_occ(int kind) { return kind == ESR_MLP_RADIANCE ? 1 : 2; }
+
+template <int KIND, typename IO>
+__device__ __forceinline__ void split_fwd_body(SplitBatch AB, IO io)
+{
+    using S = SplitSteps<KIND>;
+    constexpr NetDesc D = net_desc(KIND);
+    constexpr SplitLayout L = S::L;
+    constexpr PackLayout L32 = pack_layout(KIND);
+    constexpr int NL = S::NL, NHID = NL - 1, HT = D.hid_tiles, KS1 = L.ks[0], NS = S::NS;
+    constexpr unsigned HBYTES = HT * 32 * 32 * 4, MBYTES = (HT / 2) * 256;
+    static_assert((NL == 4 || NL == 2) && HT % 2 == 0, "the four-layer nets (radiance, BRDF, emission) and the tone mapper");
+    SplitSeg A = AB.seg[0];
+#pragma unroll
+    for (int k = 1; k < MAX_SPLIT_SEG; ++k)
+        if (k < AB.nseg && (int)blockIdx.x >= AB.seg[k].b0) A = AB.seg[k];
+    const int blk0 = A.b0, nblk = A.nb;
+    extern __shared__ __attribute__((aligned(16))) unsigned char wl[];
+    float *bias_l = reinterpret_cast<float *>(wl + S::WBYTES);
+    const int tid = threadIdx.x, lane = tid & 63, h = lane >> 5, s_ = lane & 31;
+    const int wv = __builtin_amdgcn_readfirstlane(tid >> 6);
+    const int ntiles = A.t1 - A.t0, ngroups = (ntiles + SPW - 1) / SPW;
+    for (int i = tid; i < NL * S::BIAS_FLOATS; i += 64 * SPW) {
+        const int l = i / S::BIAS_FLOATS, k = i % S::BIAS_FLOATS;
+        bias_l[i] = k < L32.tiles_out[l] * 32 ? A.packed32[L32.off_bf[l] + k] : 0.f;
+    }
+    const rsrc_t WP = make_rsrc(A.planes, (unsigned)(L.total_chunks * 1024));
+    u32x4 pre[S::PRE];
+    auto stage_load = [&](auto ST) __attribute__((always_inline)) {
+        constexpr int st = decltype(ST)::value, pieces = S::chunks(st) * 64, base = S::chunk0(st) * 1024;
+#pragma unroll
+        for (int k = 0; k < S::PRE; ++k)
+            if (k * 64 * SPW < pieces) pre[k] = __builtin_amdgcn_raw_buffer_load_b128(WP, (tid + 64 * SPW * k) * 16, base, 0);
+    };
+    auto stage_store = [&](auto ST, unsigned char *dst) __attribute__((always_inline)) {
+        constexpr int st = decltype(ST)::value, pieces = S::chunks(st) * 64;
+#pragma unroll
+        for (int k = 0; k < S::PRE; ++k)
+            if (k * 64 * SPW < pieces && tid + 64 * SPW * k < pieces)
+                *reinterpret_cast<u32x4 *>(dst + (size_t)(tid + 64 * SPW * k) * 16) = pre[k];
+    };
+    auto stage_piece = [&](auto ST, auto KC, unsigned char *dst) __attribute__((always_inline)) {
+        constexpr int st = decltype(ST)::value, k = decltype(KC)::value, pieces = S::chunks(st) * 64;
+        if constexpr (k * 64 * SPW < pieces)
+            if (tid + 64 * SPW * k < pieces) *reinterpret_cast<u32x4 *>(dst + (size_t)(tid + 64 * SPW * k) * 16) = pre[k];
+    };
+    if constexpr (S::RES) {
+        for (int i = tid; i < L.total_chunks * 64; i += 64 * SPW)
+            *reinterpret_cast<u32x4 *>(wl + (size_t)i * 16) = __builtin_amdgcn_raw_buffer_load_b128(WP, i * 16, S::BASE_CHUNK * 1024, 0);
+    } else {
+        stage_load(std::integral_constant<int, 0>{});
+        stage_store(std::integral_constant<int, 0>{}, wl);
+    }
+    step_barrier();
+
+    float xn[KS1 * 8];
+    auto fetch = [&](int tg) {
+        const int tt = A.t0 + tg * SPW + wv;
+        io.template fetch_x<KIND>(AB, A, tt < A.t1 ? tt : A.t1 - 1, tt < A.t1, h, s_, xn);
+    };
+    constexpr bool PREFETCH_X = split_occ(KIND) == 1;
+    constexpr int WR = PREFETCH_X ? WRING : 2;
+    if (PREFETCH_X && (int)blockIdx.x - blk0 < ngroups) fetch((int)blockIdx.x - blk0);
+    const int hvoff = tile_voff(lane);
+
+    int rmax = 0;
+    for (int tg = (int)blockIdx.x - blk0, trip = 0; tg < ngroups; tg += nblk, ++trip) {
+        const int par = (NS & 1) ? (trip & 1) : 0;
+        const int tt = A.t0 + tg * SPW + wv;
+        const bool live = tt < A.t1;
+        const int t = live ? tt : A.t1 - 1;
+        const bool save = A.save && live;
+        int hv = hvoff;
+        asm volatile("" : "+v"(hv));
+        f16x8 xi1[KS1], xi2[KS1], pa1[2 * HT], pa2[2 * HT], pb1[2 * HT], pb2[2 * HT];
+        if constexpr (!PREFETCH_X) fetch(tg);
+        float xmax = 0.f;
+#pragma unroll
+        for (int j = 0; j < KS1; ++j) {
+            float v[8];
+#pragma unroll
+            for (int i = 0; i < 8; ++i) v[i] = xn[j * 8 + i];
+#pragma unroll
+            for (int i = 0; i < 8; i += 2) xmax = fmaxf(xmax, fmaxf(fabsf(v[i]), fabsf(v[i + 1])));
+            split8(v, xi1[j], xi2[j]);
+        }
+        rmax = max(rmax, __float_as_int(xmax));
+        ESR_SPLIT_STAMP(0);
+        if constexpr (PREFETCH_X) fetch(tg + nblk < ngroups ? tg + nblk : tg);
+        f32x16 am[2];
+        float4 bz4[2][4];
+        float ev[16];
+        unsigned mword = 0;
+        const f32x16 zero16 = {0.f, 0.f, 0.f, 0.f, 0.f, 0.f, 0.f, 0.f, 0.f, 0.f, 0.f, 0.f, 0.f, 0.f, 0.f, 0.f};
+        const unsigned hrec = (save && A.save == 1) ? HBYTES : 0u, mrec = save ? MBYTES : 0u;
+
+        auto micro = [&](auto LC, auto IT, auto MS, f32x16 &accm, auto &o1, auto &o2) __attribute__((always_inline)) {
+            constexpr int l = decltype(LC)::value, it = decltype(IT)::value, ms = decltype(MS)::value, p = ms / 3, q = ms % 3;
+            constexpr int r0 = 2 * p, jj = r0 >> 3, i0 = r0 & 7;
+            if constexpr (q == 0) {
+                const float4 b4 = bz4[it & 1][p >> 1];
+                const float bx = (p & 1) ? b4.z : b4.x, by = (p & 1) ? b4.w : b4.y;
+                float v0 = fmaf(accm[r0], SPLIT_W_INV, bx), v1 = fmaf(accm[r0 + 1], SPLIT_W_INV, by);
+                const int b0 = __float_as_int(v0), b1 = __float_as_int(v1);
+                v0 = __int_as_float(b0 > 0 ? b0 : 0);
+                v1 = __int_as_float(b1 > 0 ? b1 : 0);
+                asm volatile("v_max3_i32 %0, %0, %1, %2" : "+v"(rmax) : "v"(__float_as_int(v0)), "v"(__float_as_int(v1)));
+                const rsrc_t RH = make_rsrc(AB.H[l] + (size_t)t * (HBYTES / 4), hrec);
+                asm volatile("" : "+v"(hv));
+                bstore1_nt(RH, v0, hv + tile_soff(0, r0), it * 4096);
+                bstore1_nt(RH, v1, hv + tile_soff(0, r0 + 1), it * 4096);
+                ev[r0] = v0; ev[r0 + 1] = v1;
+            } else if constexpr (q == 1) {
+                const float v0 = ev[r0], v1 = ev[r0 + 1];
+                int one0, one1;
+                asm volatile("v_med3_i32 %1, %3, 0, 1\n\t"
+                             "v_med3_i32 %2, %4, 0, 1\n\t"
+                             "v_lshl_or_b32 %0, %1, %5, %0\n\t"
+                             "v_lshl_or_b32 %0, %2, %6, %0"
+                             : "+v"(mword), "=&v"(one0), "=&v"(one1)
+                             : "v"(__float_as_int(v0)), "v"(__float_as_int(v1)), "n"((it & 1) * 16 + r0), "n"((it & 1) * 16 + r0 + 1));
+                put_pair<i0>(o1[2 * it + jj], v0, v1);
+            } else {
+                put_residual_pair<i0>(o2[2 * it + jj], o1[2 * it + jj], ev[r0], ev[r0 + 1]);
+            }
+        };
+        auto pending = [&](auto LC, auto IT, auto U, auto NAVAILC, f32x16 &accm, auto &o1, auto &o2) __attribute__((always_inline)) {
+            constexpr int u = decltype(U)::value, navail = decltype(NAVAILC)::value;
+            static_assert(navail >= 3 && navail % 3 == 0, "whole register pairs per pass");
+            if constexpr (u < navail)
+                sfor<0, (24 + navail - 1) / navail>([&](auto KC) {
+                    constexpr int msi = u + decltype(KC)::value * navail;
+                    if constexpr (msi < 24) micro(LC, IT, std::integral_constant<int, msi>{}, accm, o1, o2);
+                });
+            constexpr int l = decltype(LC)::value, it = decltype(IT)::value;
+            if constexpr (u == (navail < 24 ? navail : 24) - 1 && (it & 1)) {
+                __builtin_amdgcn_raw_buffer_store_b32(mword, make_rsrc(AB.M[l] + (size_t)t * (MBYTES / 4), mrec), lane * 4,
+                                                      (it >> 1) * 256, 0);
+                mword = 0;
+            }
+        };
+
+        auto run_layer = [&](auto LC, auto &in1, auto &in2, auto &o1, auto &o2) __attribute__((always_inline)) {
+            constexpr int l = decltype(LC)::value, KS = L.ks[l], NT = L.tiles_out[l], NP = L.pairs[l];
+            constexpr int s0 = [] { int s = 0; for (int k = 0; k < l; ++k) s += L.pairs[k]; return s; }();
+            constexpr bool LAST = l == NL - 1;
+            f32x16 zm;
+            sfor<0, NP>([&](auto PC) {
+                constexpr int p = decltype(PC)::value, st = s0 + p, tin = S::tiles_in(st), nxt_st = (st + 1) % NS;
+                const unsigned char *wsrc = S::RES ? wl + (S::chunk0(st) - S::BASE_CHUNK) * 1024 : wl + ((st + par) & 1) * S::BUF;
+                const u32x4 *mine = reinterpret_cast<const u32x4 *>(wsrc) + lane;
+                if constexpr (!S::RES) stage_load(std::integral_constant<int, nxt_st>{});
+                constexpr int NTOT = tin * KS;
+                u32x4 wb[WR][2];
+                sfor<0, (WR - 1 < NTOT ? WR - 1 : NTOT)>([&](auto NC) {
+                    constexpr int n0 = decltype(NC)::value, t0_ = n0 / KS, j0_ = n0 % KS;
+                    wb[n0][0] = mine[((t0_ * 2 + 0) * KS + j0_) * 64];
+                    wb[n0][1] = mine[((t0_ * 2 + 1) * KS + j0_) * 64];
+                });
+                sfor<0, NTOT>([&](auto NC) {
+                    constexpr int n = decltype(NC)::value, tt_ = n / KS, j = n % KS, it = 2 * p + tt_;
+                    if constexpr (n + WR - 1 < NTOT) {
+                        constexpr int t2 = (n + WR - 1) / KS, j2 = (n + WR - 1) % KS;
+                        wb[(n + WR - 1) % WR][0] = mine[((t2 * 2 + 0) * KS + j2) * 64];
+                        wb[(n + WR - 1) % WR][1] = mine[((t2 * 2 + 1) * KS + j2) * 64];
+                    }
+                    if constexpr (j == 0 && !LAST && PREFETCH_X) {
+                        const float4 *bp = reinterpret_cast<const float4 *>(bias_l + l * S::BIAS_FLOATS + it * 32 + (lane >> 5) * 16);
+#pragma unroll
+                        for (int q = 0; q < 4; ++q) bz4[it & 1][q] = bp[q];
+                    }
+                    f32x16 &m = LAST ? zm : am[it & 1];
+                    const f16x8 w1 = __builtin_bit_cast(f16x8, wb[n % WR][0]), w2 = __builtin_bit_cast(f16x8, wb[n % WR][1]);
+                    constexpr bool HAVE = it > 0 || l > 0;
+                    constexpr int pl = it > 0 ? l : l - 1, pit = it > 0 ? it - 1 : (l > 0 ? L.tiles_out[l > 0 ? l - 1 : 0] - 1 : 0);
+                    if constexpr (j == 0 && HAVE && !PREFETCH_X) {
+                        const float4 *bp = reinterpret_cast<const float4 *>(bias_l + pl * S::BIAS_FLOATS + pit * 32 + (lane >> 5) * 16);
+#pragma unroll
+                        for (int q = 0; q < 4; ++q) bz4[pit & 1][q] = bp[q];
+                    }
+                    auto ride = [&](auto U) __attribute__((always_inline)) {
+                        if constexpr (HAVE) {
+                            if constexpr (it > 0) pending(std::integral_constant<int, pl>{}, std::integral_constant<int, pit>{}, U,
+                                                          std::integral_constant<int, 3 * KS>{}, am[pit & 1], o1, o2);
+                            else pending(std::integral_constant<int, pl>{}, std::integral_constant<int, pit>{}, U,
+                                         std::integral_constant<int, 3 * (KS - 2)>{}, am[pit & 1], in1, in2);
+                        }
+                        if constexpr (tt_ == tin - 1 && !S::RES) {
+                            constexpr int u_ = decltype(U)::value, first = 3 * KS - S::PRE;
+                            static_assert(first >= 0, "a tile has a slot for every staged piece");
+                            if constexpr (u_ >= first) stage_piece(std::integral_constant<int, nxt_st>{}, std::integral_constant<int, u_ - first>{},
+                                                                   wl + ((st + 1 + par) & 1) * S::BUF);
+                        }
+                        __builtin_amdgcn_sched_barrier(0);
+                    };
+                    m = mfma_h(w1, in2[j], j == 0 ? zero16 : m);
+                    ride(std::integral_constant<int, 3 * j + 0>{});
+                    m = mfma_h(w1, in1[j], m);
+                    ride(std::integral_constant<int, 3 * j + 1>{});
+                    m = mfma_h(w2, in1[j], m);
+                    ride(std::integral_constant<int, 3 * j + 2>{});
+                });
+                if constexpr (LAST) {
+                    const float4 bz = *reinterpret_cast<const float4 *>(bias_l + l * S::BIAS_FLOATS + (lane >> 5) * 16);
+                    const float bzv[4] = {bz.x, bz.y, bz.z, bz.w};
+                    const rsrc_t RZ = make_rsrc(A.zout + (size_t)t * D.zrows * 32, live ? D.zrows * 32 * 4 : 0);
+                    const int zvoff = (4 * h * 32 + s_) * 4;
+#pragma unroll
+                    for (int q = 0; q < 4; ++q)
+                        bstore1(RZ, 4 * h + q < D.out_dim ? fmaf(zm[q], SPLIT_W_INV, bzv[q]) : 0.f, zvoff, q * 128);
+                }
+                ESR_SPLIT_STAMP(1 + 3 * st);
+                ESR_SPLIT_STAMP(2 + 3 * st);
+                if constexpr (!S::RES) step_barrier();
+                ESR_SPLIT_STAMP(3 + 3 * st);
+            });
+        };
+        run_layer(std::integral_constant<int, 0>{}, xi1, xi2, pa1, pa2);
+        if constexpr (NL == 4) {
+            run_layer(std::integral_constant<int, 1>{}, pa1, pa2, pb1, pb2);
+            run_layer(std::integral_constant<int, 2>{}, pb1, pb2, pa1, pa2);
+        }
+        run_layer(std::integral_constant<int, NL - 1>{}, pa1, pa2, pb1, pb2);
+    }
+    if (AB.range && rmax >= __float_as_int(SPLIT_RANGE)) atomicOr(AB.range, 1u);
+}
+
+struct DSplitSeg {
+    const _Float16 *planes;
+    int t0, t1;
+    int b0, nb;
+};
+struct DSplitBatch {
+    const float *dz;
+    const unsigned *M[3];
+    float *dZ[3];
+    float *dX;
+    float *amax;
+    int nseg;
+    DSplitSeg seg[2];
+};
+
+template <int KIND, typename IO>
+__device__ __forceinline__ void split_dgrad_body(DSplitBatch AB, IO io)
+{
+    using S = SplitSteps<KIND, true>;
+    constexpr NetDesc D = net_desc(KIND);
+    constexpr SplitLayout L = S::L;
+    constexpr int NL = S::NL, NHID = NL - 1, HT = D.hid_tiles, NS = S::NS;
+    constexpr unsigned HBYTES = HT * 32 * 32 * 4, MBYTES = (HT / 2) * 256;
+    static_assert((NL == 4 || NL == 2) && HT % 2 == 0 && L.ks[0] == 1 && L.tiles_out[NL - 1] == 2 && D.out_dim <= 8 && D.zrows <= 8,
+                  "the four-layer nets and the tone mapper: outputs in one k-step, grid-fed input rows in two tiles");
+    DSplitSeg A = AB.seg[0];
+    if (AB.nseg > 1 && (int)blockIdx.x >= AB.seg[1].b0) A = AB.seg[1];
+    const int blk0 = A.b0, nblk = A.nb;
+    extern __shared__ __attribute__((aligned(16))) unsigned char wl[];
+    const int tid = threadIdx.x, lane = tid & 63, h = lane >> 5, s_ = lane & 31;
+    const int wv = __builtin_amdgcn_readfirstlane(tid >> 6);
+    const int ntiles = A.t1 - A.t0, ngroups = (ntiles + SPW - 1) / SPW;
+    const rsrc_t WP = make_rsrc(A.planes, (unsigned)((S::BASE_CHUNK + L.total_chunks) * 1024));
+    u32x4 pre[S::PRE];
+    auto stage_load = [&](auto ST) __attribute__((always_inline)) {
+        constexpr int st = decltype(ST)::value, pieces = S::chunks(st) * 64, base = S::chunk0(st) * 1024;
+#pragma unroll
+        for (int k = 0; k < S::PRE; ++k)
+            if (k * 64 * SPW < pieces) pre[k] = __builtin_amdgcn_raw_buffer_load_b128(WP, (tid + 64 * SPW * k) * 16, base, 0);
+    };
+    auto stage_store = [&](auto ST, unsigned char *dst) __attribute__((always_inline)) {
+        constexpr int st = decltype(ST)::value, pieces = S::chunks(st) * 64;
+#pragma unroll
+        for (int k = 0; k < S::PRE; ++k)
+            if (k * 64 * SPW < pieces && tid + 64 * SPW * k < pieces)
+                *reinterpret_cast<u32x4 *>(dst + (size_t)(tid + 64 * SPW * k) * 16) = pre[k];
+    };
+    auto stage_piece = [&](auto ST, auto KC, unsigned char *dst) __attribute__((always_inline)) {
+        constexpr int st = decltype(ST)::value, k = decltype(KC)::value, pieces = S::chunks(st) * 64;
+        if constexpr (k * 64 * SPW < pieces)
+            if (tid + 64 * SPW * k < pieces) *reinterpret_cast<u32x4 *>(dst + (size_t)(tid + 64 * SPW * k) * 16) = pre[k];
+    };
+    if constexpr (S::RES) {
+        for (int i = tid; i < L.total_chunks * 64; i += 64 * SPW)
+            *reinterpret_cast<u32x4 *>(wl + (size_t)i * 16) = __builtin_amdgcn_raw_buffer_load_b128(WP, i * 16, S::BASE_CHUNK * 1024, 0);
+    } else {
+        stage_load(std::integral_constant<int, 0>{});
+        stage_store(std::integral_constant<int, 0>{}, wl);
+    }
+    step_barrier();
+
+    float zn[D.zrows];
+    unsigned mn[NHID][HT / 2];
+    auto fetch = [&](int tg) {
+        const int tt = A.t0 + tg * SPW + wv;
+        const int t = tt < A.t1 ? tt : A.t1 - 1;
+        const rsrc_t RZ = make_rsrc(AB.dz + (size_t)t * D.zrows * 32, D.zrows * 32 * 4);
+#pragma unroll
+        for (int i = 0; i < D.zrows; ++i) zn[i] = bload1(RZ, s_ * 4, i * 128);
+#pragma unroll
+        for (int l = 0; l < NHID; ++l)
+            load_relu_mask<HT>(make_rsrc(AB.M[l] + (size_t)t * (MBYTES / 4), MBYTES), mn[l], lane);
+    };
+    if ((int)blockIdx.x - blk0 < ngroups) fetch((int)blockIdx.x - blk0);
+    const int hvoff = tile_voff(lane);
+
+    float wmax = 0.f;
+    const float *gainp = reinterpret_cast<const float *>(A.planes + (size_t)(S::BASE_CHUNK + L.total_chunks) * 512);
+    const int gbits = __builtin_amdgcn_readfirstlane(__float_as_int(*gainp));
+    const int kbase = __builtin_amdgcn_readfirstlane(141 + 127 - ((gbits >> 23) & 0xff) - ((gbits & 0x7fffff) ? 1 : 0));
+    for (int tg = (int)blockIdx.x - blk0, trip = 0; tg < ngroups; tg += nblk, ++trip) {
+        const int par = (NS & 1) ? (trip & 1) : 0;
+        const int tt = A.t0 + tg * SPW + wv;
+        const bool live = tt < A.t1;
+        const int t = live ? tt : A.t1 - 1;
+        int hv = hvoff;
+        asm volatile("" : "+v"(hv));
+        typename IO::State ios;
+        if constexpr (!IO::STORE_DX) io.template group_begin<KIND>(ios, t, h, s_);
+        float zmax = 0.f;
+#pragma unroll
+        for (int i = 0; i < D.out_dim; ++i) zmax = fmaxf(zmax, fabsf(zn[i]));
+#pragma unroll
+        for (int o = 16; o > 0; o >>= 1) zmax = fmaxf(zmax, __shfl_xor(zmax, o));
+        if (live) wmax = fmaxf(wmax, zmax);
+        const int ez = (__float_as_int(zmax) >> 23) & 0xff;
+        const int ks = ez == 0 ? 0 : kbase - ez;
+        const int kc = ks < -100 ? -100 : (ks > 100 ? 100 : ks);
+        const float sc = __int_as_float((127 + kc) << 23), isc = __int_as_float((127 - kc) << 23);
+        f16x8 xi1[1], xi2[1];
+        {
+            float v[8];
+#pragma unroll
+            for (int i = 0; i < 8; ++i) v[i] = (h == 0 && i < D.out_dim) ? zn[i < D.out_dim ? i : 0] * sc : 0.f;
+            split8(v, xi1[0], xi2[0]);
+        }
+        unsigned msk[NHID][HT / 2];
+#pragma unroll
+        for (int l = 0; l < NHID; ++l)
+#pragma unroll
+            for (int w = 0; w < HT / 2; ++w) msk[l][w] = mn[l][w];
+        fetch(tg + nblk < ngroups ? tg + nblk : tg);
+        f16x8 pa1[2 * HT], pa2[2 * HT], pb1[2 * HT], pb2[2 * HT];
+        f32x16 am[2];
+        float ev[16];
+        const float wisc = SPLIT_W_INV * isc;
+        const f32x16 zero16 = {0.f, 0.f, 0.f, 0.f, 0.f, 0.f, 0.f, 0.f, 0.f, 0.f, 0.f, 0.f, 0.f, 0.f, 0.f, 0.f};
+
+        auto micro = [&](auto QC, auto IT, auto MS, f32x16 &accm, auto &o1, auto &o2) __attribute__((always_inline)) {
+            constexpr int q = decltype(QC)::value, it = decltype(IT)::value, ms = decltype(MS)::value, p = ms / 3, ph = ms % 3;
+            constexpr int r0 = 2 * p, jj = r0 >> 3, i0 = r0 & 7;
+            if constexpr (q == NL - 1) {
+                if constexpr (ph == 0 && IO::STORE_DX) {
+                    const float v0 = accm[r0] * wisc, v1 = accm[r0 + 1] * wisc;
+                    const rsrc_t RX = make_rsrc(AB.dX + (size_t)t * 64 * 32, live ? dx_rows(KIND) / 4 * 4 * 128 + (dx_rows(KIND) % 4 ? 512 : 0) : 0);
+                    asm volatile("" : "+v"(hv));
+                    bstore1(RX, v0, hv + tile_soff(0, r0), it * 4096);
+                    bstore1(RX, v1, hv + tile_soff(0, r0 + 1), it * 4096);
+                } else if constexpr (ph == 0) {
+                    io.template dx_pair<KIND, it, r0>(ios, h, accm[r0] * wisc, accm[r0 + 1] * wisc);
+                }
+            } else {
+                constexpr int d = NHID - 1 - q;
+                if constexpr (ph == 0) {
+                    int k0, k1;
+                    asm("v_bfe_i32 %0, %1, %2, 1" : "=v"(k0) : "v"(msk[d][it >> 1]), "n"((it & 1) * 16 + r0));
+                    asm("v_bfe_i32 %0, %1, %2, 1" : "=v"(k1) : "v"(msk[d][it >> 1]), "n"((it & 1) * 16 + r0 + 1));
+                    const int a0 = __float_as_int(accm[r0]) & k0, a1 = __float_as_int(accm[r0 + 1]) & k1;
+                    const rsrc_t RD = make_rsrc(AB.dZ[d] + (size_t)t * (HBYTES / 4), (live && AB.dZ[d]) ? HBYTES : 0u);
+                    asm volatile("" : "+v"(hv));
+                    bstore1_nt(RD, __int_as_float(a0) * wisc, hv + tile_soff(0, r0), it * 4096);
+                    bstore1_nt(RD, __int_as_float(a1) * wisc, hv + tile_soff(0, r0 + 1), it * 4096);
+                    ev[r0] = __int_as_float(a0) * SPLIT_W_INV; ev[r0 + 1] = __int_as_float(a1) * SPLIT_W_INV;
+                } else if constexpr (ph == 1) {
+                    put_pair<i0>(o1[2 * it + jj], ev[r0], ev[r0 + 1]);
+                } else {
+                    put_residual_pair<i0>(o2[2 * it + jj], o1[2 * it + jj], ev[r0], ev[r0 + 1]);
+                }
+            }
+        };
+        auto pending = [&](auto QC, auto IT, auto U, auto NAVAILC, f32x16 &accm, auto &o1, auto &o2) __attribute__((always_inline)) {
+            constexpr int u = decltype(U)::value, navail = decltype(NAVAILC)::value;
+            static_assert(navail >= 3 && navail % 3 == 0, "whole register pairs per pass");
+            if constexpr (u < navail)
+                sfor<0, (24 + navail - 1) / navail>([&](auto KC) {
+                    constexpr int msi = u + decltype(KC)::value * navail;
+                    if constexpr (msi < 24) micro(QC, IT, std::integral_constant<int, msi>{}, accm, o1, o2);
+                });
+        };
+        auto run_layer = [&](auto QC, auto &in1, auto &in2, auto &o1, auto &o2) __attribute__((always_inline)) {
+            constexpr int q = decltype(QC)::value, KS = L.ks[q], NT = L.tiles_out[q], NP = L.pairs[q];
+            constexpr int s0 = [] { int s = 0; for (int k = 0; k < q; ++k) s += L.pairs[k]; return s; }();
+            sfor<0, NP>([&](auto PC) {
+                constexpr int p = decltype(PC)::value, st = s0 + p, tin = S::tiles_in(st), nxt_st = (st + 1) % NS;
+                const unsigned char *wsrc = S::RES ? wl + (S::chunk0(st) - S::BASE_CHUNK) * 1024 : wl + ((st + par) & 1) * S::BUF;
+                const u32x4 *mine = reinterpret_cast<const u32x4 *>(wsrc) + lane;
+                if constexpr (!S::RES) stage_load(std::integral_constant<int, nxt_st>{});
+                constexpr int NTOT = tin * KS;
+                u32x4 wb[WRING][2];
+                sfor<0, (WRING - 1 < NTOT ? WRING - 1 : NTOT)>([&](auto NC) {
+                    constexpr int n0 = decltype(NC)::value, t0_ = n0 / KS, j0_ = n0 % KS;
+                    wb[n0][0] = mine[((t0_ * 2 + 0) * KS + j0_) * 64];
+                    wb[n0][1] = mine[((t0_ * 2 + 1) * KS + j0_) * 64];
+                });
+                sfor<0, NTOT>([&](auto NC) {
+                    constexpr int n = decltype(NC)::value, tt_ = n / KS, j = n % KS, it = 2 * p + tt_;
+                    if constexpr (n + WRING - 1 < NTOT) {
+                        constexpr int t2 = (n + WRING - 1) / KS, j2 = (n + WRING - 1) % KS;
+                        wb[(n + WRING - 1) % WRING][0] = mine[((t2 * 2 + 0) * KS + j2) * 64];
+                        wb[(n + WRING - 1) % WRING][1] = mine[((t2 * 2 + 1) * KS + j2) * 64];
+                    }
+                    f32x16 &m = am[it & 1];
+                    const f16x8 w1 = __builtin_bit_cast(f16x8, wb[n % WRING][0]), w2 = __builtin_bit_cast(f16x8, wb[n % WRING][1]);
+                    constexpr bool HAVE = it > 0 || q > 0;
+                    constexpr int pq = it > 0 ? q : q - 1, pit = it > 0 ? it - 1 : (q > 0 ? L.tiles_out[q > 0 ? q - 1 : 0] - 1 : 0);
+                    auto ride = [&](auto U) __attribute__((always_inline)) {
+                        if constexpr (HAVE) {
+                            if constexpr (it > 0) pending(std::integral_constant<int, pq>{}, std::integral_constant<int, pit>{}, U,
+                                                          std::integral_constant<int, 3 * KS>{}, am[pit & 1], o1, o2);
+                            else pending(std::integral_constant<int, pq>{}, std::integral_constant<int, pit>{}, U,
+                                         std::integral_constant<int, 3 * (KS - 2)>{}, am[pit & 1], in1, in2);
+                        }
+                        if constexpr (tt_ == tin - 1 && 3 * KS >= S::PRE && !S::RES) {
+                            constexpr int u_ = decltype(U)::value, first = 3 * KS - S::PRE;
+                            if constexpr (u_ >= first) stage_piece(std::integral_constant<int, nxt_st>{}, std::integral_constant<int, u_ - first>{},
+                                                                   wl + ((st + 1 + par) & 1) * S::BUF);
+                        }
+                        __builtin_amdgcn_sched_barrier(0);
+                    };
+                    m = mfma_h(w1, in2[j], j == 0 ? zero16 : m);
+                    ride(std::integral_constant<int, 3 * j + 0>{});
+                    m = mfma_h(w1, in1[j], m);
+                    ride(std::integral_constant<int, 3 * j + 1>{});
+                    m = mfma_h(w2, in1[j], m);
+                    ride(std::integral_constant<int, 3 * j + 2>{});
+                });
+                if constexpr (q == NL - 1 && p == NP - 1) {
+                    sfor<0, 24>([&](auto MC) {
+                        micro(QC, std::integral_constant<int, NT - 1>{}, MC, am[(NT - 1) & 1], o1, o2);
+                    });
+                }
+                if constexpr (3 * KS < S::PRE && !S::RES)
+                    stage_store(std::integral_constant<int, nxt_st>{}, wl + ((st + 1 + par) & 1) * S::BUF);
+                if constexpr (!S::RES) step_barrier();
+            });
+        };
+        run_layer(std::integral_constant<int, 0>{}, xi1, xi2, pa1, pa2);
+        if constexpr (NL == 4) {
+            run_layer(std::integral_constant<int, 1>{}, pa1, pa2, pb1, pb2);
+            run_layer(std::integral_constant<int, 2>{}, pb1, pb2, pa1, pa2);
+        }
+        run_layer(std::integral_constant<int, NL - 1>{}, pa1, pa2, pb1, pb2);
+        if constexpr (!IO::STORE_DX) io.template group_end<KIND>(ios, t, live, h, s_);
+    }
+    wmax *= fmaxf(1.f, *gainp * 0.0625f);
+    if (AB.amax && lane == 0 && wmax > *reinterpret_cast<volatile float *>(AB.amax))
+        atomicMax(reinterpret_cast<unsigned *>(AB.amax), __float_as_uint(wmax));
+}
+
+struct SplitLoadX {
+    template <int KIND, int N>
+    __device__ __forceinline__ void fetch_x(const SplitBatch &AB, const SplitSeg &A, int t, bool, int h, int s_, float (&xn)[N]) const
+    {
+        constexpr NetDesc D = net_desc(KIND);
+        constexpr int KS1 = N / 8;
+        const rsrc_t RX = make_rsrc(AB.X + (size_t)t * D.xrows * 32, D.xrows * 32 * 4);
+        const int xvoff = (h * 8 * 32 + s_) * 4, coff = A.crow * 128;
+#pragma unroll
+        for (int j = 0; j < KS1; ++j)
+#pragma unroll
+            for (int i = 0; i < 8; ++i) {
+                const int row = 16 * j + 8 * h + i;
+                xn[j * 8 + i] = bload1(RX, xvoff + (row < D.cw ? coff : 0), (16 * j + i) * 128);
+            }
+    }
+};
+
+struct SplitStoreDX {
+    static constexpr bool STORE_DX = true;
+    struct State {};
+    template <int KIND> __device__ void group_begin(State &, int, int, int) const {}
+    template <int KIND, int it, int r0> __device__ void dx_pair(State &, int, float, float) const {}
+    template <int KIND> __device__ void group_end(State &, int, bool, int, int) const {}
+};
+
+}
diff --git a/esr_nerf_amd/fine_engine.py b/esr_nerf_amd/fine_engine.py
--- a/esr_nerf_amd/fine_engine.py
+++ b/esr_nerf_amd/fine_engine.py
@@ -154,6 +154,7 @@
         self.x16 = self.bf16
         self.split_fwd = (not self.bf16) and os.environ.get("ESR_SPLIT_FWD", "1") != "0"
         self.split_strict = os.environ.get("ESR_SPLIT_STRICT", "0") == "1"
+        self.tone_fused = os.environ.get("ESR_TONE_FUSED", "1") != "0"
         self.split_fallback_steps = 0
         self.packed_split: Dict[str, torch.Tensor] = {}
         self._psplit = {}
@@ -243,6 +244,9 @@
             with self.f32_only():
                 out = (rerun or run)()
         return out
+
+    def _tone_fused(self):
+        return self.tone_fused and not self.bf16 and self.split_fwd and "tone" in self.packed_split
 
     def _run(self, name, fn, *args):
         self.n_calls += 1
@@ -484,9 +488,9 @@
                       _lib.ptr(ws["X16"]) if x16 else None, tiles_on, tiles_all, H, M, 88, _lib.ptr(ws["z_off"]),
                       _lib.ptr(ws["z_emo"]), s)
         self._run("tone_in_fwd", L.esr_fine_tone_in_fwd, _lib.ptr(ws["z_off"]), _lib.ptr(ws["z_emo"]), tiles_on, tiles_all,
-                                          _lib.ptr(ws["lin"]), _lib.ptr(ws["Xt"]), s)
+                  _lib.ptr(ws["lin"]), _lib.ptr(ws["Xt"]), s)
         self._run("mlp_fwd(tone)", self.mlp_fwd, KIND_TONEMAP, _lib.ptr(self.packed["tone"]), _lib.ptr(ws["Xt"]), 0, tiles_all,
-                                 self._H(["Ht"]), self._H(["Mt"]), 2, 0, _lib.ptr(ws["zt"]), s)
+                  self._H(["Ht"]), self._H(["Mt"]), 2, 0, _lib.ptr(ws["zt"]), s)
         self.range_probe()
         self._run("composite_fwd", L.esr_fine_composite_fwd, _lib.ptr(ws["zt"]), _lib.ptr(ws["lin"]), _lib.ptr(ws["rec_ray"]),
                                             _lib.ptr(ws["rec_w"]), tiles_all, _lib.ptr(ws["rgb"]),
@@ -651,15 +655,20 @@
         if self.bf16:
             self._run("mlp_dgrad(tone)", L.esr_mlp_dgrad_bf16, KIND_TONEMAP, self._p16[self.packed["tone"].data_ptr()],
                       _lib.ptr(ws["dzt"]), 0, ta, self._H(["Mt"]), dZt_arg, _lib.ptr(ws["dXt"]), s)
+        elif split and self._tone_fused():
+            self._run("mlp_dgrad(tone)", L.esr_tone_fused_bwd, _lib.ptr(self.packed_split["tone"]), _lib.ptr(ws["dzt"]), _lib.ptr(ws["Mt"]),
+                      _lib.ptr(ws["Xt"]), _lib.ptr(g_lin), _lib.ptr(ws["z_off"]), _lib.ptr(ws["z_emo"]), _lib.ptr(ws["rec_ray"]),
+                      _lib.ptr(ws["rec_w"]), to, ta, _lib.ptr(ws["dz"]), _lib.ptr(ctx.amax_t), s)
         elif split:
             self._run("mlp_dgrad(tone)", L.esr_mlp_dgrad_split, KIND_TONEMAP, _lib.ptr(self.packed_split["tone"]), _lib.ptr(ws["dzt"]),
                       0, ta, self._H(["Mt"]), dZt_arg, _lib.ptr(ws["dXt"]), _lib.ptr(ctx.amax_t), s)
         else:
             self._run("mlp_dgrad(tone)", L.esr_mlp_dgrad, KIND_TONEMAP, _lib.ptr(self.packed["tone"]), _lib.ptr(ws["dzt"]), 0, ta,
                       self._H(["Mt"]), dZt_arg, _lib.ptr(ws["dXt"]), s)
-        self._run("tone_in_bwd", L.esr_fine_tone_in_bwd, _lib.ptr(ws["dXt"]), _lib.ptr(ws["Xt"]), _lib.ptr(g_lin), _lib.ptr(ws["lin"]),
-                  _lib.ptr(ws["z_off"]), _lib.ptr(ws["z_emo"]), _lib.ptr(ws["rec_ray"]), _lib.ptr(ws["rec_w"]), to, ta,
-                  _lib.ptr(ws["dz"]), s)
+        if not (split and self._tone_fused()):
+            self._run("tone_in_bwd", L.esr_fine_tone_in_bwd, _lib.ptr(ws["dXt"]), _lib.ptr(ws["Xt"]), _lib.ptr(g_lin), _lib.ptr(ws["lin"]),
+                      _lib.ptr(ws["z_off"]), _lib.ptr(ws["z_emo"]), _lib.ptr(ws["rec_ray"]), _lib.ptr(ws["rec_w"]), to, ta,
+                      _lib.ptr(ws["dz"]), s)
         if self.bf16:
             pe, po = self.packed["emo"].data_ptr(), self.packed["off"].data_ptr()
             self._run("mlp_dgrad(rad)", L.esr_mlp_dgrad_fine_bf16, self._p16[pe], self._p16[po],
diff --git a/include/esr_hip.h b/include/esr_hip.h
--- a/include/esr_hip.h
+++ b/include/esr_hip.h
@@ -12,7 +12,7 @@
 
 #define ESR_TILE 32
 
-#define ESR_ABI_VERSION 29
+#define ESR_ABI_VERSION 30
 int esr_abi_version(void);
 const char *esr_build_info(void);
 
@@ -205,6 +205,11 @@
                         float *const *dZ, float *dX, float *amax, void *stream);
 int esr_mlp_dgrad_fine_split(const void *planes_emo, const void *planes_off, const float *dz, int32_t t_on, int32_t t_all,
                              const uint32_t *const *M, float *const *dZ, float *dX, float *amax, void *stream);
+int esr_tone_fused_fwd(const float *packed32, const void *planes, const float *z_off, const float *z_emo, int32_t tiles_on,
+                       int32_t tiles_all, uint32_t *Mt, float *lin, float *Xt, float *zt, void *stream);
+int esr_tone_fused_bwd(const void *planes, const float *dzt, const uint32_t *Mt, const float *Xt, const float *g_lin,
+                       const float *z_off, const float *z_emo, const int32_t *rec_ray, const float *rec_w, int32_t tiles_on,
+                       int32_t tiles_all, float *dz, float *amax, void *stream);
 int esr_absmax(const float *x, int64_t n, float *out, void *stream);
 
 int esr_mlp_fwd(int kind, const float *packed, const float *X, int32_t t0, int32_t t1,
```
